# PlanNoa/video_super_resolution

Hardware: AMD Instinct MI355X
Metric: HR frames/sec, 1080p->4K x4 VSR (LR 540x960 -> 2160x3840), VSR.forward end-to-end (higher is better)
Workload: dtype f16

## Files before the change

### __graft_entry__.py

```python
import os

os.environ.setdefault("MIOPEN_FIND_MODE", "2")
os.environ.setdefault("MIOPEN_DEBUG_ENABLE_AI_IMMED_MODE_FALLBACK", "0")
os.environ.setdefault("MIOPEN_LOG_LEVEL", "2")
import subprocess
import sys

ROOT = os.path.dirname(os.path.abspath(__file__))
if ROOT not in sys.path:
    sys.path.insert(0, ROOT)


def build() -> None:
    from video_super_resolution_amd import _lib
    _lib.build(verbose=True)
    subprocess.check_call(["make", "-s", "-C", os.path.join(ROOT, "oracle"), "_build/liboracle_native.so"])
    import video_super_resolution_amd
    missing = [s for s in _lib.declared_symbols() if not hasattr(_lib.load(), s)]
    if missing:
        raise RuntimeError(f"libvsr_hip.so lacks {missing}")
    xmissing = [s for s in _lib.declared_symbols() + _lib.declared_symbols(xcheck=True) if not hasattr(_lib.load_xcheck(), s)]
    if xmissing:
        raise RuntimeError(f"libvsr_hip_xcheck.so lacks {xmissing}")
    s3missing = [s for s in _lib.declared_symbols(s3=True) if not hasattr(_lib.load_s3(), s)]
    if s3missing:
        raise RuntimeError(f"libvsr_hip_s3.so lacks {s3missing}")
    s3tmissing = [s for s in _lib.declared_symbols(s3t=True) if not hasattr(_lib.load_s3t(), s)]
    if s3tmissing:
        raise RuntimeError(f"libvsr_hip_s3t.so lacks {s3tmissing}")
    s3pmissing = [s for s in _lib.declared_symbols(s3p=True) if not hasattr(_lib.load_s3p(), s)]
    if s3pmissing:
        raise RuntimeError(f"libvsr_hip_s3p.so lacks {s3pmissing}")
    s3fmissing = [s for s in _lib.declared_symbols(s3f=True) if not hasattr(_lib.load_s3f(), s)]
    if s3fmissing:
        raise RuntimeError(f"libvsr_hip_s3f.so lacks {s3fmissing}")
    yuvmissing = [s for s in _lib.declared_symbols(yuv=True) if not hasattr(_lib.load_yuv(), s)]
    if yuvmissing:
        raise RuntimeError(f"libvsr_hip_yuv.so lacks {yuvmissing}")
    metricmissing = [s for s in _lib.declared_symbols(metric=True) if not hasattr(_lib.load_metric(), s)]
    if metricmissing:
        raise RuntimeError(f"libvsr_hip_metric.so lacks {metricmissing}")
    optmissing = [s for s in _lib.declared_symbols(opt=True) if not hasattr(_lib.load_opt(), s)]
    if optmissing:
        raise RuntimeError(f"libvsr_hip_opt.so lacks {optmissing}")
    lossmissing = [s for s in _lib.declared_symbols(loss=True) if not hasattr(_lib.load_loss(), s)]
    if lossmissing:
        raise RuntimeError(f"libvsr_hip_loss.so lacks {lossmissing}")
    resizemissing = [s for s in _lib.declared_symbols(resize=True) if not hasattr(_lib.load_resize(), s)]
    if resizemissing:
        raise RuntimeError(f"libvsr_hip_resize.so lacks {resizemissing}")
    warpmissing = [s for s in _lib.declared_symbols(warp=True) if not hasattr(_lib.load_warp(), s)]
    if warpmissing:
        raise RuntimeError(f"libvsr_hip_warp.so lacks {warpmissing}")
    scenemissing = [s for s in _lib.declared_symbols(scene=True) if not hasattr(_lib.load_scene(), s)]
    if scenemissing:
        raise RuntimeError(f"libvsr_hip_scene.so lacks {scenemissing}")
    hgimissing = [s for s in _lib.declared_symbols(hgi=True) if not hasattr(_lib.load_hgi(), s)]
    if hgimissing:
        raise RuntimeError(f"libvsr_hip_hgi.so lacks {hgimissing}")
    msssimmissing = [s for s in _lib.declared_symbols(msssim=True) if not hasattr(_lib.load_msssim(), s)]
    if msssimmissing:
        raise RuntimeError(f"libvsr_hip_msssim.so lacks {msssimmissing}")
    pixmissing = [s for s in _lib.declared_symbols(pix=True) if not hasattr(_lib.load_pix(), s)]
    if pixmissing:
        raise RuntimeError(f"libvsr_hip_pix.so lacks {pixmissing}")
    patchmissing = [s for s in _lib.declared_symbols(patch=True) if not hasattr(_lib.load_patch(), s)]
    if patchmissing:
        raise RuntimeError(f"libvsr_hip_patch.so lacks {patchmissing}")
    deintmissing = [s for s in _lib.declared_symbols(deint=True) if not hasattr(_lib.load_deint(), s)]
    if deintmissing:
        raise RuntimeError(f"libvsr_hip_deint.so lacks {deintmissing}")
    cellmissing = [s for s in _lib.declared_symbols(cell=True) if not hasattr(_lib.load_cell(), s)]
    if cellmissing:
        raise RuntimeError(f"libvsr_hip_cell.so lacks {cellmissing}")


def smoke() -> None:
    import numpy as np
    import torch
    from oracle import native, vsr_oracle
    from video_super_resolution_amd import SRProjectionModule, ops
    from video_super_resolution_amd.weights import fill_module_

    assert torch.cuda.is_available(), "smoke() needs cuda:0"
    torch.cuda.set_device(0)
    rs = np.random.RandomState(0)
    img = rs.randn(1, 3, 32, 48).astype(np.float32)
    flow = (rs.randn(1, 2, 32, 48) * 4).astype(np.float32)
    got = ops.resample2d(torch.from_numpy(img).cuda(), torch.from_numpy(flow).cuda()).cpu().numpy()
    assert np.array_equal(got, native.resample2d(img, flow)), "flow warp differs from the oracle"

    from video_super_resolution_amd import frames as F
    red = rs.randint(0, 256, (2, 20, 24)).astype(np.int64)
    rgb = np.zeros((2, 20, 24, 3), dtype=np.float32)
    rgb[..., 0] = red
    cells = F.cell_stats(torch.from_numpy(rgb).cuda(), luma4=(1.0, 0.0, 0.0, 0.0)).cpu().numpy()
    act = np.zeros_like(red)
    act[:, :, :-1] += np.abs(red[:, :, :-1] - red[:, :, 1:])
    act[:, :-1] += np.abs(red[:, :-1] - red[:, 1:])
    assert cells.shape == (2, 2, 2, 2) and cells[0, 0, 0, 0] == act[0, :16, :16].sum() and cells[1, 1, 1, 0] == act[1, 16:, 16:].sum(), \
        "cell activity differs from the sum it restates"
    assert not cells[0, :, :, 1].any() and cells[1, :, :, 1].sum() == np.abs(red[1] - red[0]).sum(), "cell temporal sums differ"

    sr = fill_module_(SRProjectionModule().eval(), seed=0, prefix="model.")
    x = torch.from_numpy(rs.randint(0, 256, (8, 3, 10, 12)).astype(np.float32))
    with torch.no_grad():
        ref = vsr_oracle.sr_forward({k: v for k, v in sr.state_dict().items()}, x).numpy()
    sr = sr.cuda()
    errs = {}
    for precision, bar in (("fp32", 1e-3), ("fp16", 5e-3)):
        sr.precision = precision
        out = sr(x.cuda()).cpu().numpy()
        errs[precision] = np.abs(out - ref).max() / np.abs(ref).max()
        assert errs[precision] < bar, f"SR forward ({precision}) differs from the oracle: {errs[precision]}"
    print(f"smoke ok: warp bit-exact, SR forward rel err fp32 {errs['fp32']:.2e}, fp16/MFMA {errs['fp16']:.2e}")


if __name__ == "__main__":
    build()
    if len(sys.argv) > 1 and sys.argv[1] == "smoke":
        smoke()
```

### video_super_resolution_amd/_lib.py

```python
from __future__ import annotations

import ctypes
import os
import re
import subprocess

import torch

_PKG = os.path.dirname(os.path.abspath(__file__))
_ROOT = os.path.dirname(_PKG)
LIB_PATH = os.path.join(_PKG, "libvsr_hip.so")
XLIB_PATH = os.path.join(_PKG, "libvsr_hip_xcheck.so")
HEADER_PATH = os.path.join(_ROOT, "include", "vsr_hip.h")
XHEADER_PATH = os.path.join(_ROOT, "include", "vsr_hip_xcheck.h")
_lib = None
_xlib = None


def _side(name: str, prefix: str, abi: int, has_query: bool) -> tuple:
    return (os.path.join(_PKG, f"libvsr_hip_{name}.so"), os.path.join(_ROOT, "include", f"vsr_hip_{name}.h"), prefix, abi, has_query)


_SIDE = {"grad": _side("grad", "vsr_grad", 1, False), "s3": _side("s3", "vsr_s3", 1, True), "s3t": _side("s3t", "vsr_s3t", 1, True),
         "s3p": _side("s3p", "vsr_s3p", 1, True), "s3f": _side("s3f", "vsr_s3f", 1, True), "yuv": _side("yuv", "vsr_yuv", 1, False),
         "metric": _side("metric", "vsr_metric", 1, False), "opt": _side("opt", "vsr_opt", 1, False), "loss": _side("loss", "vsr_loss", 1, False),
         "resize": _side("resize", "vsr_resize", 1, False), "warp": _side("warp", "vsr_warp", 1, False),
         "scene": _side("scene", "vsr_scene", 1, False), "hgi": _side("hgi", "vsr_hgi", 1, False),
         "msssim": _side("msssim", "vsr_msssim", 1, False), "pix": _side("pix", "vsr_pix", 1, False),
         "patch": _side("patch", "vsr_patch", 1, False), "deint": _side("deint", "vsr_deint", 1, False),
         "cell": _side("cell", "vsr_cell", 1, False)}
(GLIB_PATH, GHEADER_PATH), (S3LIB_PATH, S3HEADER_PATH), (S3TLIB_PATH, S3THEADER_PATH), (S3PLIB_PATH, S3PHEADER_PATH), \
    (S3FLIB_PATH, S3FHEADER_PATH), (YUVLIB_PATH, YUVHEADER_PATH), (METRICLIB_PATH, METRICHEADER_PATH), (OPTLIB_PATH, OPTHEADER_PATH), \
    (LOSSLIB_PATH, LOSSHEADER_PATH), (RESIZELIB_PATH, RESIZEHEADER_PATH), (WARPLIB_PATH, WARPHEADER_PATH), (SCENELIB_PATH, SCENEHEADER_PATH), \
    (HGILIB_PATH, HGIHEADER_PATH), (MSSSIMLIB_PATH, MSSSIMHEADER_PATH), (PIXLIB_PATH, PIXHEADER_PATH), (PATCHLIB_PATH, PATCHHEADER_PATH), \
    (DEINTLIB_PATH, DEINTHEADER_PATH), (CELLLIB_PATH, CELLHEADER_PATH) = (row[:2] for row in _SIDE.values())
_gradlib = _s3lib = _s3tlib = _s3plib = _s3flib = _yuvlib = _metriclib = _optlib = _losslib = _resizelib = _warplib = _scenelib = _hgilib = _msssimlib = _pixlib = _patchlib = _deintlib = _celllib = None
_use_x = os.environ.get("VSR_USE_XCHECK", "0") == "1" or bool(os.environ.get("VSR_TUNING", "").strip())


class VsrHipError(RuntimeError):
    pass


def build(verbose: bool = False) -> str:
    cmd = ["make", "-j4", "-C", os.path.join(_PKG, "csrc")]
    if not verbose:
        cmd.insert(1, "-s")
    subprocess.check_call(cmd)
    return LIB_PATH


def declared_symbols(xcheck: bool = False, grad: bool = False, s3: bool = False, s3t: bool = False, s3p: bool = False, s3f: bool = False,
                     yuv: bool = False, metric: bool = False, opt: bool = False, loss: bool = False, resize: bool = False,
                     warp: bool = False, scene: bool = False, hgi: bool = False, msssim: bool = False, pix: bool = False,
                     patch: bool = False, deint: bool = False, cell: bool = False) -> list:
    side = [name for name, on in (("grad", grad), ("s3", s3), ("s3t", s3t), ("s3p", s3p), ("s3f", s3f), ("yuv", yuv), ("metric", metric),
                                  ("opt", opt), ("loss", loss), ("resize", resize), ("warp", warp), ("scene", scene), ("hgi", hgi),
                                  ("msssim", msssim), ("pix", pix), ("patch", patch), ("deint", deint), ("cell", cell)) if on]
    with open(_SIDE[side[-1]][1] if side else XHEADER_PATH if xcheck else HEADER_PATH) as f:
        text = re.sub(r"/\*.*?\*/", "", f.read(), flags=re.S)
    return sorted(set(re.findall(r"\b(vsr_[a-z0-9_]+)\s*\(", text)))


def _dlopen(path: str) -> ctypes.CDLL:
    if not os.path.exists(path):
        raise VsrHipError(
            f"{path} is missing: build it with `python -c 'import __graft_entry__ as g; g.build()'` "
            "(there is no CPU fallback for the device path)")
    return ctypes.CDLL(path)


def _open(path: str) -> ctypes.CDLL:
    lib = _dlopen(path)
    lib.vsr_last_error.restype = ctypes.c_char_p
    lib.vsr_last_route.restype = ctypes.c_char_p
    for fn in ("vsr_sr_query", "vsr_train_corr_dw_ws_floats", "vsr_train_prelu_bwd_ws_floats"):
        getattr(lib, fn).restype = ctypes.c_size_t
    if lib.vsr_abi_version() != 3:
        raise VsrHipError(f"{os.path.basename(path)}: ABI version mismatch")
    return lib


def load_xcheck() -> ctypes.CDLL:
    global _xlib
    if _xlib is None:
        lib = _open(XLIB_PATH)
        for t in os.environ.get("VSR_TUNING", "").split(","):
            if t.strip():
                lib.vsr_conv2d_tuning(int(t))
        _xlib = lib
    return _xlib


def _load_side(name: str) -> ctypes.CDLL:
    cache = f"_{name}lib"
    if globals()[cache] is None:
        path, _, prefix, abi, has_query = _SIDE[name]
        lib = _dlopen(path)
        getattr(lib, prefix + "_last_error").restype = ctypes.c_char_p
        lib.vsr_last_error = getattr(lib, prefix + "_last_error")
        if has_query:
            getattr(lib, prefix + "_query").restype = ctypes.c_size_t
        if getattr(lib, prefix + "_abi_version")() != abi:
            raise VsrHipError(f"{os.path.basename(path)}: ABI version mismatch")
        globals()[cache] = lib
    return globals()[cache]


def load_grad() -> ctypes.CDLL:
    return _load_side("grad")


def load_s3() -> ctypes.CDLL:
    return _load_side("s3")


def load_s3t() -> ctypes.CDLL:
    return _load_side("s3t")


def load_s3p() -> ctypes.CDLL:
    return _load_side("s3p")


def load_s3f() -> ctypes.CDLL:
    return _load_side("s3f")


def load_yuv() -> ctypes.CDLL:
    return _load_side("yuv")


def load_metric() -> ctypes.CDLL:
    lib = _load_side("metric")
    lib.vsr_metric_ws_bytes.restype = ctypes.c_size_t
    return lib


class OptTensor(ctypes.Structure):
    _fields_ = [("p", ctypes.c_void_p), ("g", ctypes.c_void_p), ("m", ctypes.c_void_p), ("v", ctypes.c_void_p), ("n", ctypes.c_ulonglong)]


def load_opt() -> ctypes.CDLL:
    lib = _load_side("opt")
    lib.vsr_opt_plan_bytes.restype = lib.vsr_opt_norm_ws_bytes.restype = ctypes.c_size_t
    lib.vsr_opt_plan_bytes.argtypes = [ctypes.c_int, ctypes.POINTER(ctypes.c_ulonglong)]
    lib.vsr_opt_plan_fill.argtypes = [ctypes.c_void_p, ctypes.c_size_t, ctypes.c_int, ctypes.POINTER(OptTensor)]
    lib.vsr_opt_norm_ws_bytes.argtypes = [ctypes.c_void_p]
    lib.vsr_opt_adam_f32.argtypes = [ctypes.c_void_p] * 3 + [ctypes.c_float] * 7 + [ctypes.c_void_p]
    lib.vsr_opt_grad_norm.argtypes = [ctypes.c_void_p, ctypes.c_void_p, ctypes.c_double, ctypes.c_void_p, ctypes.c_void_p, ctypes.c_void_p]
    return lib


def load_loss() -> ctypes.CDLL:
    lib = _load_side("loss")
    lib.vsr_loss_ws_bytes.restype = ctypes.c_size_t
    lib.vsr_loss_ws_bytes.argtypes = [ctypes.c_int, ctypes.c_int]
    lib.vsr_loss_pixel_terms.argtypes = [ctypes.c_void_p] * 3 + [ctypes.c_int] * 2 + [ctypes.c_void_p] * 6
    return lib


def load_resize() -> ctypes.CDLL:
    lib = _load_side("resize")
    lib.vsr_resize_frames.argtypes = [ctypes.c_void_p] * 2 + [ctypes.c_int] * 5 + [ctypes.c_void_p, ctypes.c_void_p, ctypes.c_int] * 2 + \
        [ctypes.c_int, ctypes.c_void_p]
    return lib


def load_warp() -> ctypes.CDLL:
    lib = _load_side("warp")
    lib.vsr_warp_ws_bytes.restype = ctypes.c_size_t
    lib.vsr_warp_ws_bytes.argtypes = [ctypes.c_int] * 4
    lib.vsr_warp_error.argtypes = [ctypes.c_void_p] * 2 + [ctypes.c_int] * 7 + [ctypes.c_void_p] * 2 + [ctypes.c_int] + [ctypes.c_longlong] * 3 + \
        [ctypes.c_int] * 3 + [ctypes.c_void_p] * 5
    return lib


def load_scene() -> ctypes.CDLL:
    lib = _load_side("scene")
    lib.vsr_scene_ws_bytes.restype = ctypes.c_size_t
    lib.vsr_scene_ws_bytes.argtypes = [ctypes.c_int] * 3
    lib.vsr_scene_pair_sums.argtypes = [ctypes.c_void_p] * 2 + [ctypes.c_int] * 3 + [ctypes.c_void_p] * 4
    lib.vsr_scene_decide.argtypes = [ctypes.c_void_p, ctypes.c_int, ctypes.c_void_p, ctypes.c_double, ctypes.c_double, ctypes.c_void_p, ctypes.c_void_p]
    lib.vsr_scene_window.argtypes = [ctypes.c_void_p] * 4 + [ctypes.c_int] * 2 + [ctypes.c_void_p] * 4 + [ctypes.c_int] * 2 + [ctypes.c_void_p]
    return lib


def load_hgi() -> ctypes.CDLL:
    lib = _load_side("hgi")
    lib.vsr_hgi_workgroups.restype = ctypes.c_longlong
    lib.vsr_hgi_inception_f16.argtypes = [ctypes.c_void_p] + [ctypes.c_int] * 3 + [ctypes.c_void_p] * 2 + [ctypes.c_int] * 3 + \
        [ctypes.c_void_p, ctypes.c_void_p, ctypes.c_int] * 3 + [ctypes.c_int, ctypes.c_void_p] + [ctypes.c_int] * 4 + [ctypes.c_void_p]
    return lib


def load_msssim() -> ctypes.CDLL:
    lib = _load_side("msssim")
    lib.vsr_msssim_ws_bytes.restype = ctypes.c_size_t
    lib.vsr_msssim_ws_bytes.argtypes = [ctypes.c_int] * 5
    lib.vsr_msssim_frames.argtypes = [ctypes.c_void_p] * 2 + [ctypes.c_int] * 6 + [ctypes.c_void_p] * 5
    return lib


def load_pix() -> ctypes.CDLL:
    return _load_side("pix")


def load_patch() -> ctypes.CDLL:
    lib = _load_side("patch")
    lib.vsr_patch_gather.argtypes = [ctypes.c_void_p] + [ctypes.c_int] * 3 + [ctypes.c_void_p, ctypes.c_int, ctypes.c_void_p] + \
        [ctypes.c_int] * 4 + [ctypes.c_void_p] * 3
    return lib


class DeintPlane(ctypes.Structure):
    _fields_ = [("offset", ctypes.c_size_t), ("rows", ctypes.c_int), ("cols", ctypes.c_int), ("comps", ctypes.c_int)]


def load_deint() -> ctypes.CDLL:
    lib = _load_side("deint")
    lib.vsr_deint_frame.argtypes = [ctypes.c_void_p] * 4 + [ctypes.POINTER(DeintPlane)] + [ctypes.c_int] * 5 + [ctypes.c_void_p]
    return lib


def load_cell() -> ctypes.CDLL:
    lib = _load_side("cell")
    lib.vsr_cell_stats.argtypes = [ctypes.c_void_p] + [ctypes.c_int] * 3 + [ctypes.c_void_p] * 3
    return lib


def load() -> ctypes.CDLL:
    global _lib
    if _use_x:
        return load_xcheck()
    if _lib is None:
        _lib = _open(LIB_PATH)
    return _lib


class xcheck:

    def __enter__(self):
        global _use_x
        self._old, _use_x = _use_x, True
        return load_xcheck()

    def __exit__(self, *exc):
        global _use_x
        _use_x = self._old
        return False


Q_UTD_BLOB_BYTES, Q_UTD_STRIP_WIDTH, Q_UTD_S2_BLOB_BYTES, Q_UTD_S2_STRIP_WIDTH, Q_TAIL_S2_BLOB_BYTES = range(5)
Q_S3_BLOB_BYTES, Q_S3_STRIP_WIDTH = range(2)
Q_S3T_BLOB_BYTES, Q_S3T_BLOB_FOLD_BYTES, Q_S3T_STRIP_WIDTH = range(3)
Q_S3P_BLOB_BYTES, Q_S3P_STRIP_WIDTH = range(2)
Q_S3F_BLOB_BYTES, Q_S3F_STRIP_WIDTH = range(2)


def check(rc: int, what: str = "", lib=None) -> None:
    if rc != 0:
        libs = [lib] if lib is not None else [l for l in (load(), _lib, _xlib) if l is not None]
        msgs = []
        for l in libs:
            m = l.vsr_last_error().decode("utf-8", "replace")
            if m and m not in msgs:
                msgs.append(m)
        raise VsrHipError(f"{what or 'vsr'} failed ({rc}): {' | '.join(msgs)}")


def dptr(t: torch.Tensor, dtype=torch.float32) -> ctypes.c_void_p:
    if not t.is_cuda:
        raise VsrHipError("device path called with a CPU tensor (no CPU fallback exists)")
    if t.dtype != dtype:
        raise VsrHipError(f"expected {dtype}, got {t.dtype}")
    if not t.is_contiguous():
        raise VsrHipError("tensor must be contiguous")
    return ctypes.c_void_p(t.data_ptr())


def optr(t, dtype=torch.float32):
    return ctypes.c_void_p(0) if t is None else dptr(t, dtype)


_raw_stream = getattr(torch._C, "_cuda_getCurrentRawStream", None)


def raw_stream(index=None) -> int:
    if _raw_stream is not None:
        return _raw_stream(torch._C._cuda_getDevice() if index is None else index)
    return torch.cuda.current_stream(index).cuda_stream


def stream() -> ctypes.c_void_p:
    return ctypes.c_void_p(raw_stream())


def _first_cuda_tensor(objs):
    for o in objs:
        if isinstance(o, torch.Tensor):
            if o.is_cuda:
                return o
        elif isinstance(o, (list, tuple)):
            t = _first_cuda_tensor(o)
            if t is not None:
                return t
    return None


def on_device(fn):
    import functools

    @functools.wraps(fn)
    def wrapped(*args, **kwargs):
        t = _first_cuda_tensor(args)
        if t is None:
            t = _first_cuda_tensor(tuple(kwargs.values()))
        if t is None or t.device.index == torch.cuda.current_device():
            return fn(*args, **kwargs)
        with torch.cuda.device(t.device):
            return fn(*args, **kwargs)
    return wrapped


def cf(v: float) -> ctypes.c_float:
    return ctypes.c_float(float(v))


class _ChainStage(ctypes.Structure):
    _fields_ = [("inp", ctypes.c_void_p * 2), ("w", ctypes.c_void_p * 2), ("ldw", ctypes.c_int * 2), ("w_prev", ctypes.c_void_p),
                ("ldw_prev", ctypes.c_int), ("bias", ctypes.c_void_p), ("cmap", ctypes.c_void_p), ("slope", ctypes.c_float),
                ("out", ctypes.c_void_p)]


class Chain1x1(ctypes.Structure):
    _fields_ = [("nstages", ctypes.c_int), ("stage", _ChainStage * 3)]


_ROUTE_BATCH = os.environ.get("VSR_ROUTE_BATCH", "1") != "0"


class route_batch:

    def __init__(self, num: int, den: int):
        self.num, self.den = int(num), int(den)
        self.on = self.den > 0 and self.num > 0 and self.num != self.den and _ROUTE_BATCH

    def __enter__(self):
        if self.on:
            check(load().vsr_conv2d_route_batch(self.num, self.den), "conv2d_route_batch")
        return self

    def __exit__(self, *exc):
        if self.on:
            load().vsr_conv2d_route_batch(0, 0)
        return False


class serial_streams:
    on = False

    def __init__(self, enable: bool = True):
        self.enable = bool(enable)

    def __enter__(self):
        self._old, serial_streams.on = serial_streams.on, serial_streams.on or self.enable
        return self

    def __exit__(self, *exc):
        serial_streams.on = self._old
        return False


class EventTimer:

    def __init__(self):
        self.enabled = False
        self.only = None
        self._pairs = {}

    def reset(self):
        self._pairs = {}

# ... 47 lines not shown
```

### video_super_resolution_amd/csrc/conv_igemm.hip

```cpp
#include "conv_common.h"
#include "conv_kwalk.h"
#include "conv_patch.h"

namespace {

using vsrc::h8;
using vsrc::h4;
using vsrc::f4;
using vsrc::BM;
using vsrc::ConvP;
using vsrc::sw_off;
using vsrc::u4;
using vsrc::u2;
using vsrc::dma16;
using vsrc::patch_epilogue;
using vsrc::patch_epilogue_act;
using vsrc::patch_pixoff;
using vsrc::stage_patch;
using vsrc::patch_pieces;
using vsrc::stage_patch_cached;
using vsrc::PT_H;
using vsrc::PT_W;

struct C0 { static constexpr int value = 0; };
struct C1 { static constexpr int value = 1; };
struct C2 { static constexpr int value = 2; };
struct C3 { [[maybe_unused]] static constexpr int value = 3; };
struct C4 { [[maybe_unused]] static constexpr int value = 4; };


template <int BN, int ACT>
__device__ __forceinline__ void gather_store(const ConvP& p, const f4 (&acc)[BN / 16][2], long long M, long long m0, int co0, int tid, int zsplit,
                                             int ph, int oy_off, int ox_off) {
    constexpr int MT = BN / 16;
    const int lane = tid & 63, wv = tid >> 6, l15 = lane & 15, g = lane >> 4;
    if (p.splits > 1) {
#pragma unroll
        for (int nt = 0; nt < 2; ++nt) {
            const long long m = m0 + 32 * wv + 16 * nt + l15;
            if (m >= M) continue;
            float* wsp = p.ws + (((size_t)zsplit * (p.nphase > 1 ? 4 : 1) + ph) * M + m) * p.cout_pad + co0;
#pragma unroll
            for (int mt = 0; mt < MT; ++mt) *reinterpret_cast<f4*>(wsp + 16 * mt + 4 * g) = acc[mt][nt];
        }
        return;
    }
    f4 bz[MT];
#pragma unroll
    for (int mt = 0; mt < MT; ++mt)
        bz[mt] = p.bias ? *reinterpret_cast<const f4*>(p.bias + co0 + 16 * mt + 4 * g) : f4{0.0f, 0.0f, 0.0f, 0.0f};
    const bool vec_ok = (p.out_coff & 3) == 0 && (p.out_ld & 3) == 0;
    const unsigned HoWo = (unsigned)(p.Ho * p.Wo);
#pragma unroll
    for (int nt = 0; nt < 2; ++nt) {
        const long long m = m0 + 32 * wv + 16 * nt + l15;
        if (m >= M) continue;
        const int n = (int)((unsigned)m / HoWo);
        const int rem = (int)((unsigned)m - (unsigned)n * HoWo);
        const int oy = rem / p.Wo, ox = rem - oy * p.Wo;
        _Float16* dst = p.out + (((size_t)n * p.outH + oy * p.oy_mul + oy_off) * p.outW + ox * p.ox_mul + ox_off) * p.out_ld +
                        p.out_coff;
#pragma unroll
        for (int mt = 0; mt < MT; ++mt) {
            const int c = co0 + 16 * mt + 4 * g;
            if (c >= p.cout) continue;
            float v[4];
#pragma unroll
            for (int r = 0; r < 4; ++r) {
                float t = acc[mt][nt][r] + bz[mt][r];
                if (ACT == 1) t = fmaxf(t, 0.0f);
                else if (ACT == 2) t = t >= 0.0f ? t : t * p.slope;
                v[r] = t;
            }
            if (vec_ok && c + 4 <= p.cout) {
                *reinterpret_cast<h4*>(dst + c) = h4{(_Float16)v[0], (_Float16)v[1], (_Float16)v[2], (_Float16)v[3]};
            } else {
#pragma unroll
                for (int r = 0; r < 4; ++r)
                    if (c + r < p.cout) dst[c + r] = (_Float16)v[r];
            }
        }
    }
}

#if VSR_X
template <int BN, bool STEM = false>
__global__ void __launch_bounds__(256) k_conv_igemm(const ConvP p) {
    constexpr int MT = BN / 16;
    constexpr int A_HALF = BN * 64;
    constexpr int B_HALF = BM * 64;
    constexpr int STAGE = 2 * (A_HALF + B_HALF);
    constexpr int A_PIECES = A_HALF / 16;
    constexpr int AP = (A_PIECES + 255) / 256;
    extern __shared__ __attribute__((aligned(16))) unsigned char smem[];
    auto As = [&](int b, int hf) __attribute__((always_inline)) { return smem + b * STAGE + hf * (A_HALF + B_HALF); };
    auto Bs = [&](int b, int hf) __attribute__((always_inline)) { return smem + b * STAGE + hf * (A_HALF + B_HALF) + A_HALF; };
    u4* const tab = reinterpret_cast<u4*>(smem + 2 * STAGE);

    const int tid = threadIdx.x, lane = tid & 63, wv = tid >> 6;
    const int l15 = lane & 15, g = lane >> 4;
    const long long M = (long long)p.N * p.Ho * p.Wo;
    const long long m0 = (long long)blockIdx.x * BM;
    const int co0 = blockIdx.y * BN;
    const int nchunk = STEM ? 1 : p.cin >> 5;
    const int npair = STEM ? p.kh : p.kh * p.kw * nchunk;
    const int nk_all = (npair + 1) >> 1;
    const vsrc::KRange kr = vsrc::k_range(p, blockIdx.z, nk_all);
    const int ph = kr.ph, zsplit = kr.zsplit, pad_y = kr.pad_y, pad_x = kr.pad_x, oy_off = kr.oy_off, ox_off = kr.ox_off;
    const int ks_per = kr.ks_per, ks0 = kr.ks0, nk = kr.nk;
    const _Float16* const wpk = kr.wpk;

    const __amdgpu_buffer_rsrc_t w_rsrc = vsrc::kwalk_w_rsrc(p, wpk, npair), in_rsrc = vsrc::kwalk_in_rsrc(p);

    vsrc::build_kwalk<STEM>(p, tab, tid, ks0, nk, npair, nchunk, vsrc::kwalk_entries(ks_per, vsrc::KWALK_FIRST_LOOKAHEAD));

    const int bchunk = tid & 3;
    const int brow[2] = {tid >> 2, (tid + 256) >> 2};
    int piy0[2], pix0[2];
    unsigned pbase[2];
    bool xok0[2], xok1[2];
#pragma unroll
    for (int r = 0; r < 2; ++r) {
        const vsrc::PixOrigin o = vsrc::pixel_origin<STEM>(p, m0 + brow[r], M, pad_y, pad_x, bchunk);
        piy0[r] = o.piy0; pix0[r] = o.pix0; pbase[r] = o.pbase;
        xok0[r] = (unsigned)pix0[r] < (unsigned)p.W;
        xok1[r] = (unsigned)(pix0[r] + 1) < (unsigned)p.W;
    }
    unsigned wlane[AP];
#pragma unroll
    for (int ap = 0; ap < AP; ++ap) wlane[ap] = tid + 256 * ap < A_PIECES ? (unsigned)(co0 * 64 + (tid + 256 * ap) * 16) : 0x40000000u;

    u4 ra[2][2][AP], rb[2][2][2];
    __syncthreads();
    int q = 0;
    u4 en[2] = {tab[0], tab[1]};
    auto gload = [&](auto setc) __attribute__((always_inline)) {
        constexpr int S = decltype(setc)::value;
#pragma unroll
        for (int hf = 0; hf < 2; ++hf) {
            const u4 e = en[hf];
#pragma unroll
            for (int ap = 0; ap < AP; ++ap) ra[S][hf][ap] = __builtin_amdgcn_raw_buffer_load_b128(w_rsrc, wlane[ap] + e[3], 0, 0);
#pragma unroll
            for (int r = 0; r < 2; ++r) {
                const bool rowok = (unsigned)(piy0[r] + (int)e[1]) < (unsigned)p.H;
                if (STEM) {
                    const u2 t0 = __builtin_amdgcn_raw_buffer_load_b64(in_rsrc, rowok && xok0[r] ? pbase[r] + e[0] : 0xFFFFFFFFu, 0, 0);
                    const u2 t1 = __builtin_amdgcn_raw_buffer_load_b64(in_rsrc, rowok && xok1[r] ? pbase[r] + e[0] + 8u : 0xFFFFFFFFu, 0, 0);
                    rb[S][hf][r] = u4{t0[0], t0[1], t1[0], t1[1]};
                } else {
                    const bool ok = rowok && (unsigned)(pix0[r] + (int)e[2]) < (unsigned)p.W;
                    rb[S][hf][r] = __builtin_amdgcn_raw_buffer_load_b128(in_rsrc, ok ? pbase[r] + e[0] : 0xFFFFFFFFu, 0, 0);
                }
            }
        }
// ... 61 lines not shown
    else if (p.act == 1) gather_store<BN, 1>(p, acc, M, m0, co0, tid, zsplit, ph, oy_off, ox_off);
    else gather_store<BN, 2>(p, acc, M, m0, co0, tid, zsplit, ph, oy_off, ox_off);
}
#endif


template <int BN, bool STEM = false, int D = 3>
__global__ void __launch_bounds__(256) k_conv_igemm_d(const ConvP p) {
    constexpr int MT = BN / 16;
    constexpr int A_HALF = BN * 64;
    constexpr int STAGE = 2 * A_HALF;
    constexpr int A_PIECES = A_HALF / 16;
    constexpr int AP = (A_PIECES + 255) / 256;
    extern __shared__ __attribute__((aligned(16))) unsigned char smem[];
    auto As = [&](int b, int hf) __attribute__((always_inline)) { return smem + b * STAGE + hf * A_HALF; };
    u4* const tab = reinterpret_cast<u4*>(smem + 2 * STAGE);

    const int tid = threadIdx.x, lane = tid & 63, wv = tid >> 6;
    const int l15 = lane & 15, g = lane >> 4;
    const long long M = (long long)p.N * p.Ho * p.Wo;
    const long long m0 = (long long)blockIdx.x * BM;
    const int co0 = blockIdx.y * BN;
    const int nchunk = STEM ? 1 : p.cin >> 5;
    const int npair = STEM ? p.kh : p.kh * p.kw * nchunk;
    const int nk_all = (npair + 1) >> 1;
    const vsrc::KRange kr = vsrc::k_range(p, blockIdx.z, nk_all);
    const int ph = kr.ph, zsplit = kr.zsplit, pad_y = kr.pad_y, pad_x = kr.pad_x, oy_off = kr.oy_off, ox_off = kr.ox_off;
    const int ks_per = kr.ks_per, ks0 = kr.ks0, nk = kr.nk;
    const _Float16* const wpk = kr.wpk;

    const __amdgpu_buffer_rsrc_t w_rsrc = vsrc::kwalk_w_rsrc(p, wpk, npair), in_rsrc = vsrc::kwalk_in_rsrc(p);

    vsrc::build_kwalk<STEM>(p, tab, tid, ks0, nk, npair, nchunk, vsrc::kwalk_entries(ks_per, vsrc::kwalk_gather_lookahead(D)));

    int piy0[2], pix0[2];
    unsigned pbase[2];
    bool xok0[2], xok1[2];
#pragma unroll
    for (int r = 0; r < 2; ++r) {
        const int row = 32 * wv + 16 * r + l15;
        const vsrc::PixOrigin o = vsrc::pixel_origin<STEM>(p, m0 + row, M, pad_y, pad_x, g);
        piy0[r] = o.piy0; pix0[r] = o.pix0; pbase[r] = o.pbase;
        xok0[r] = (unsigned)pix0[r] < (unsigned)p.W;
        xok1[r] = (unsigned)(pix0[r] + 1) < (unsigned)p.W;
    }

    u4 ra[D][2][AP], rb[D][2][2];
    unsigned wlane[AP];
#pragma unroll
    for (int ap = 0; ap < AP; ++ap) wlane[ap] = tid + 256 * ap < A_PIECES ? (unsigned)(co0 * 64 + (tid + 256 * ap) * 16) : 0x40000000u;
    __syncthreads();
    int q = 0;
    u4 en[2] = {tab[0], tab[1]};
    auto gload = [&](auto setc, auto setb) __attribute__((always_inline)) {
        constexpr int S = decltype(setc)::value, SB = decltype(setb)::value;
#pragma unroll
        for (int hf = 0; hf < 2; ++hf) {
            const u4 e = en[hf];
#pragma unroll
            for (int ap = 0; ap < AP; ++ap) ra[S][hf][ap] = __builtin_amdgcn_raw_buffer_load_b128(w_rsrc, wlane[ap] + e[3], 0, 0);
#pragma unroll
            for (int r = 0; r < 2; ++r) {
                const bool rowok = (unsigned)(piy0[r] + (int)e[1]) < (unsigned)p.H;
                if (STEM) {
                    const u2 t0 = __builtin_amdgcn_raw_buffer_load_b64(in_rsrc, rowok && xok0[r] ? pbase[r] + e[0] : 0xFFFFFFFFu, 0, 0);
                    const u2 t1 = __builtin_amdgcn_raw_buffer_load_b64(in_rsrc, rowok && xok1[r] ? pbase[r] + e[0] + 8u : 0xFFFFFFFFu, 0, 0);
                    rb[SB][hf][r] = u4{t0[0], t0[1], t1[0], t1[1]};
                } else {
                    const bool ok = rowok && (unsigned)(pix0[r] + (int)e[2]) < (unsigned)p.W;
                    rb[SB][hf][r] = __builtin_amdgcn_raw_buffer_load_b128(in_rsrc, ok ? pbase[r] + e[0] : 0xFFFFFFFFu, 0, 0);
                }
            }
        }
        q += 2;
        en[0] = tab[q];
        en[1] = tab[q + 1];
    };
    auto lstore = [&](int buf, auto setc) __attribute__((always_inline)) {
        constexpr int S = decltype(setc)::value;
#pragma unroll
        for (int hf = 0; hf < 2; ++hf) {
#pragma unroll
            for (int ap = 0; ap < AP; ++ap) {
                const int piece = tid + 256 * ap;
                if (piece < A_PIECES) *reinterpret_cast<u4*>(As(buf, hf) + sw_off(piece >> 2, piece & 3)) = ra[S][hf][ap];
            }
        }
    };

    f4 acc[MT][2];
#pragma unroll
    for (int mt = 0; mt < MT; ++mt)
#pragma unroll
        for (int nt = 0; nt < 2; ++nt) acc[mt][nt] = f4{0.0f, 0.0f, 0.0f, 0.0f};

    gload(C0{}, C0{});
    lstore(ks0 & 1, C0{});
    gload(C1{}, C1{});
    if constexpr (D == 5) {
        gload(C2{}, C2{});
        gload(C3{}, C3{});
    }
    __syncthreads();
    auto body = [&](int ks, auto cur, auto nxt, auto nw) __attribute__((always_inline)) {
        constexpr int BC = decltype(cur)::value;
        const int buf = ks & 1;
        h8 af[2][MT];
#pragma unroll
        for (int mt = 0; mt < MT; ++mt) af[0][mt] = *reinterpret_cast<const h8*>(As(buf, 0) + sw_off(16 * mt + l15, g));
        __builtin_amdgcn_sched_barrier(0);
        gload(nw, nw);
        __builtin_amdgcn_sched_barrier(0);
#pragma unroll
        for (int mt = 0; mt < MT; ++mt) af[1][mt] = *reinterpret_cast<const h8*>(As(buf, 1) + sw_off(16 * mt + l15, g));
        __builtin_amdgcn_sched_barrier(0);
        if (ks < nk) {
#pragma unroll
            for (int hf = 0; hf < 2; ++hf) {
                h8 bf[2];
#pragma unroll
                for (int nt = 0; nt < 2; ++nt) bf[nt] = __builtin_bit_cast(h8, rb[BC][hf][nt]);
#pragma unroll
                for (int mt = 0; mt < MT; ++mt)
#pragma unroll
                    for (int nt = 0; nt < 2; ++nt)
                        acc[mt][nt] = __builtin_amdgcn_mfma_f32_16x16x32_f16(af[hf][mt], bf[nt], acc[mt][nt], 0, 0, 0);
            }
        }
        lstore(buf ^ 1, nxt);
        __syncthreads();
    };
    if constexpr (D == 5) {
        for (int ks = ks0; ks < nk; ks += 5) {
            body(ks, C0{}, C1{}, C4{});
            body(ks + 1, C1{}, C2{}, C0{});
            body(ks + 2, C2{}, C3{}, C1{});
            body(ks + 3, C3{}, C4{}, C2{});
            body(ks + 4, C4{}, C0{}, C3{});
        }
    } else {
        for (int ks = ks0; ks < nk; ks += 3) {
            body(ks, C0{}, C1{}, C2{});
            body(ks + 1, C1{}, C2{}, C0{});
            body(ks + 2, C2{}, C0{}, C1{});
        }
    }

    if (p.splits > 1 || p.act == 0) gather_store<BN, 0>(p, acc, M, m0, co0, tid, zsplit, ph, oy_off, ox_off);
    else if (p.act == 1) gather_store<BN, 1>(p, acc, M, m0, co0, tid, zsplit, ph, oy_off, ox_off);
    else gather_store<BN, 2>(p, acc, M, m0, co0, tid, zsplit, ph, oy_off, ox_off);
}


constexpr int C1_MAX_CHUNKS = 8;
template <int NCH>
__global__ void __launch_bounds__(512) k_conv1x1_stream(const ConvP p) {
    extern __shared__ __attribute__((aligned(16))) unsigned char wsm[];
    const int tid = threadIdx.x, lane = tid & 63, wv = tid >> 6;
    const int l15 = lane & 15, g = lane >> 4;
    const long long M = (long long)p.N * p.Ho * p.Wo;
    const int rows = NCH * p.cout_pad;
    for (int q = tid; q < rows * 4; q += 512)
        *reinterpret_cast<uint4*>(wsm + sw_off(q >> 2, q & 3)) = *reinterpret_cast<const uint4*>(p.wpk + (size_t)q * 8);
    float* const bsm = reinterpret_cast<float*>(wsm + (size_t)rows * 64);
    for (int q = tid; q < p.cout_pad; q += 512) bsm[q] = (p.bias && q < p.cout) ? p.bias[q] : 0.0f;
    __syncthreads();
    const int ntile = min(p.cout_pad >> 4, 2 * ((p.cout + 31) >> 5));
    const long long nblk = (M + 255) / 256;
    h8 bf[NCH][2], nx[NCH][2];
    auto fetch = [&](long long blk, h8 (&dst)[NCH][2]) __attribute__((always_inline)) {
#pragma unroll
        for (int nt = 0; nt < 2; ++nt) {
            const long long m = blk * 256 + 32 * wv + 16 * nt + l15;
            const _Float16* src = p.in + (size_t)(m < M ? m : M - 1) * p.in_ld + p.in_coff + 8 * g;
#pragma unroll
            for (int c = 0; c < NCH; ++c) dst[c][nt] = *reinterpret_cast<const h8*>(src + 32 * c);
        }
    };
    if ((long long)blockIdx.x < nblk) fetch(blockIdx.x, nx);
    for (long long blk = blockIdx.x; blk < nblk; blk += gridDim.x) {
        const long long mbase = blk * 256 + 32 * wv;
#pragma unroll
        for (int c = 0; c < NCH; ++c)
#pragma unroll
            for (int nt = 0; nt < 2; ++nt) bf[c][nt] = nx[c][nt];
        if (blk + gridDim.x < nblk) fetch(blk + gridDim.x, nx);
        const float nslope = p.act == 1 ? 0.0f : (p.act == 2 ? p.slope : 1.0f);
        const bool vec_ok = (p.out_coff & 7) == 0 && (p.out_ld & 7) == 0;
        int t = 0;
        for (; t + 1 < ntile; t += 2) {
            const int rowA = 16 * t + 8 * (l15 >> 2) + (l15 & 3);
            h8 a0[NCH], a1[NCH];
#pragma unroll
            for (int c = 0; c < NCH; ++c) {
                a0[c] = *reinterpret_cast<const h8*>(wsm + sw_off(c * p.cout_pad + rowA, g));
                a1[c] = *reinterpret_cast<const h8*>(wsm + sw_off(c * p.cout_pad + rowA + 4, g));
            }
            const int c0 = 16 * t + 8 * g;
            const f4 b0 = *reinterpret_cast<const f4*>(bsm + c0), b1 = *reinterpret_cast<const f4*>(bsm + c0 + 4);
            f4 acc[2][2];
#pragma unroll
            for (int nt = 0; nt < 2; ++nt) { acc[0][nt] = b0; acc[1][nt] = b1; }
#pragma unroll
            for (int c = 0; c < NCH; ++c)
#pragma unroll
                for (int nt = 0; nt < 2; ++nt) {
                    acc[0][nt] = __builtin_amdgcn_mfma_f32_16x16x32_f16(a0[c], bf[c][nt], acc[0][nt], 0, 0, 0);
                    acc[1][nt] = __builtin_amdgcn_mfma_f32_16x16x32_f16(a1[c], bf[c][nt], acc[1][nt], 0, 0, 0);
                }
            const bool full = vec_ok && c0 + 8 <= p.cout;
#pragma unroll
            for (int nt = 0; nt < 2; ++nt) {
                const long long m = mbase + 16 * nt + l15;
                float v[8];
#pragma unroll
                for (int r = 0; r < 8; ++r) {
                    const float x = acc[r >> 2][nt][r & 3];
                    v[r] = fmaxf(x, 0.0f) + nslope * fminf(x, 0.0f);
                }
                _Float16* dst = p.out + (size_t)(m < M ? m : 0) * p.out_ld + p.out_coff + c0;
                if (m < M && full) {
                    *reinterpret_cast<h8*>(dst) = h8{(_Float16)v[0], (_Float16)v[1], (_Float16)v[2], (_Float16)v[3],
                                                     (_Float16)v[4], (_Float16)v[5], (_Float16)v[6], (_Float16)v[7]};
                } else if (m < M) {
#pragma unroll
                    for (int r = 0; r < 8; ++r)
                        if (c0 + r < p.cout) dst[r] = (_Float16)v[r];
                }
            }
        }
        if (t < ntile) {
            h8 a0[NCH];
#pragma unroll
            for (int c = 0; c < NCH; ++c) a0[c] = *reinterpret_cast<const h8*>(wsm + sw_off(c * p.cout_pad + 16 * t + l15, g));
            const int c0 = 16 * t + 4 * g;
            const f4 b0 = *reinterpret_cast<const f4*>(bsm + c0);
            f4 acc[2] = {b0, b0};
#pragma unroll
            for (int c = 0; c < NCH; ++c)
#pragma unroll
                for (int nt = 0; nt < 2; ++nt) acc[nt] = __builtin_amdgcn_mfma_f32_16x16x32_f16(a0[c], bf[c][nt], acc[nt], 0, 0, 0);
            const bool full = (p.out_coff & 3) == 0 && (p.out_ld & 3) == 0 && c0 + 4 <= p.cout;
#pragma unroll
            for (int nt = 0; nt < 2; ++nt) {
                const long long m = mbase + 16 * nt + l15;
                float v[4];
#pragma unroll
                for (int r = 0; r < 4; ++r) v[r] = fmaxf(acc[nt][r], 0.0f) + nslope * fminf(acc[nt][r], 0.0f);
                _Float16* dst = p.out + (size_t)(m < M ? m : 0) * p.out_ld + p.out_coff + c0;
                if (m < M && full) {
                    *reinterpret_cast<h4*>(dst) = h4{(_Float16)v[0], (_Float16)v[1], (_Float16)v[2], (_Float16)v[3]};
                } else if (m < M) {
#pragma unroll
                    for (int r = 0; r < 4; ++r)
                        if (c0 + r < p.cout) dst[r] = (_Float16)v[r];
                }
            }
        }
    }
}

#if VSR_X
constexpr int C1T_SLOT = 32 * 256;
__global__ void __launch_bounds__(256) k_conv1x1_t(const ConvP p) {
    constexpr int NCH = 4;
    extern __shared__ __attribute__((aligned(16))) unsigned char wsm[];
    const int tid = threadIdx.x, lane = tid & 63, wv = __builtin_amdgcn_readfirstlane(tid >> 6);
    const int l15 = lane & 15, g = lane >> 4;
    const long long M = (long long)p.N * p.Ho * p.Wo;
    const int rows = NCH * p.cout_pad;
    for (int q = tid; q < rows * 4; q += 256)
        *reinterpret_cast<uint4*>(wsm + sw_off(q >> 2, q & 3)) = *reinterpret_cast<const uint4*>(p.wpk + (size_t)q * 8);
    float* const bsm = reinterpret_cast<float*>(wsm + (size_t)rows * 64);
    for (int q = tid; q < p.cout_pad; q += 256) bsm[q] = (p.bias && q < p.cout) ? p.bias[q] : 0.0f;
    unsigned char* const slots = wsm + (size_t)rows * 64 + (size_t)p.cout_pad * 4 + (size_t)wv * 2 * C1T_SLOT;
    __syncthreads();
    const long long nblk = (M + 127) / 128;
    const __amdgpu_buffer_rsrc_t in_rsrc = __builtin_amdgcn_make_buffer_rsrc(
        const_cast<_Float16*>(p.in), 0, (int)((size_t)M * p.in_ld * 2), 0x00020000);
    const __amdgpu_buffer_rsrc_t out_rsrc = __builtin_amdgcn_make_buffer_rsrc(p.out, 0, (int)((size_t)M * p.out_ld * 2), 0x00020000);
    const int dq = lane >> 4, ds = lane & 15;
    auto fetch = [&](long long blk, int slot) __attribute__((always_inline)) {
        const long long m0 = blk * 128 + 32 * wv;
#pragma unroll
        for (int k = 0; k < 8; ++k) {
            const int pl = 4 * k + dq;
            const long long m = m0 + pl;
            const unsigned off = m < M ? (unsigned)(((size_t)m * p.in_ld + p.in_coff) * 2 + ((ds ^ (pl & 15)) << 4)) : 0xFFFFFFFFu;
            dma16(in_rsrc, slots + slot * C1T_SLOT + 1024 * k, off);
        }
    };
    const float nslope = p.act == 1 ? 0.0f : (p.act == 2 ? p.slope : 1.0f);
    const int ngroup = (p.cout + 127) >> 7;
    auto store_group = [&](const unsigned char* tile, long long mbase, int grp) __attribute__((always_inline)) {
        const int npair = min(4, (p.cout_pad - 128 * grp) >> 5);
        const int ch = 128 * grp + 8 * ds;
        const bool ch_ok = ch + 8 <= p.cout && ds < 4 * npair;
#pragma unroll
        for (int k = 0; k < 8; ++k) {
            const int pl = 4 * k + dq;
            const long long m = mbase + pl;
            const u4 v = *reinterpret_cast<const u4*>(tile + pl * 256 + ((ds ^ (pl & 15)) << 4));
            const unsigned off = (ch_ok && m < M) ? (unsigned)(((size_t)m * p.out_ld + p.out_coff + ch) * 2) : 0xFFFFFFFFu;
            __builtin_amdgcn_raw_buffer_store_b128(v, out_rsrc, off, 0, 0);
        }
        asm volatile("s_waitcnt lgkmcnt(0)" ::: "memory");
    };
    int cur = 0;
    bool have_prev = false;
    long long prev_mbase = 0;
    if ((long long)blockIdx.x >= nblk) return;
    fetch(blockIdx.x, 0);
    for (long long blk = blockIdx.x; blk < nblk; blk += gridDim.x, cur ^= 1) {
        unsigned char* const img = slots + cur * C1T_SLOT;
        unsigned char* const oth = slots + (cur ^ 1) * C1T_SLOT;
        asm volatile("s_waitcnt vmcnt(0)" ::: "memory");
        h8 bf[NCH][2];
#pragma unroll
        for (int nt = 0; nt < 2; ++nt)
#pragma unroll
            for (int c = 0; c < NCH; ++c) {
                const int pl = 16 * nt + l15;
                bf[c][nt] = *reinterpret_cast<const h8*>(img + pl * 256 + (((4 * c + g) ^ (pl & 15)) << 4));
            }
        asm volatile("s_waitcnt lgkmcnt(0)" ::: "memory");
        if (have_prev) store_group(oth, prev_mbase, ngroup - 1);
        fetch(blk + gridDim.x, cur ^ 1);
        const long long mbase = blk * 128 + 32 * wv;
        for (int grp = 0; grp < ngroup; ++grp) {
            const int npair = min(4, (p.cout_pad - 128 * grp) >> 5);
            for (int tp = 0; tp < npair; ++tp) {
                const int t = 8 * grp + 2 * tp;
                const int rowA = 16 * t + 8 * (l15 >> 2) + (l15 & 3);
                h8 a0[NCH], a1[NCH];
#pragma unroll
                for (int c = 0; c < NCH; ++c) {
                    a0[c] = *reinterpret_cast<const h8*>(wsm + sw_off(c * p.cout_pad + rowA, g));
                    a1[c] = *reinterpret_cast<const h8*>(wsm + sw_off(c * p.cout_pad + rowA + 4, g));
                }
                const int c0 = 16 * t + 8 * g;
                const f4 b0 = *reinterpret_cast<const f4*>(bsm + c0), b1 = *reinterpret_cast<const f4*>(bsm + c0 + 4);
                f4 acc[2][2];
#pragma unroll
                for (int nt = 0; nt < 2; ++nt) { acc[0][nt] = b0; acc[1][nt] = b1; }
#pragma unroll
                for (int c = 0; c < NCH; ++c)
#pragma unroll
                    for (int nt = 0; nt < 2; ++nt) {
                        acc[0][nt] = __builtin_amdgcn_mfma_f32_16x16x32_f16(a0[c], bf[c][nt], acc[0][nt], 0, 0, 0);
                        acc[1][nt] = __builtin_amdgcn_mfma_f32_16x16x32_f16(a1[c], bf[c][nt], acc[1][nt], 0, 0, 0);
                    }
#pragma unroll
                for (int nt = 0; nt < 2; ++nt) {
                    float v[8];
#pragma unroll
                    for (int r = 0; r < 8; ++r) {
                        const float x = acc[r >> 2][nt][r & 3];
                        v[r] = fmaxf(x, 0.0f) + nslope * fminf(x, 0.0f);
                    }
                    const int pl = 16 * nt + l15;
                    *reinterpret_cast<h8*>(img + pl * 256 + (((4 * tp + g) ^ (pl & 15)) << 4)) =
                        h8{(_Float16)v[0], (_Float16)v[1], (_Float16)v[2], (_Float16)v[3], (_Float16)v[4], (_Float16)v[5], (_Float16)v[6], (_Float16)v[7]};
                }
            }
            asm volatile("" ::: "memory");
            if (grp + 1 < ngroup) store_group(img, mbase, grp);
        }
        have_prev = true;
        prev_mbase = mbase;
    }
    store_group(slots + (cur ^ 1) * C1T_SLOT, prev_mbase, ngroup - 1);
    asm volatile("s_waitcnt vmcnt(0)" ::: "memory");
}
#endif




template <int MT>
__global__ void __launch_bounds__(256) k_conv_patch(const ConvP p) {
    extern __shared__ __attribute__((aligned(16))) unsigned char psm[];
    const int PH = PT_H + p.kh - 1, PW = PT_W + p.kw - 1;
    const int ntap = p.kh * p.kw;
    unsigned char* const patch = psm;
    const int tid = threadIdx.x, lane = tid & 63, wv = tid >> 6;
    const int l15 = lane & 15, g = lane >> 4;
    const vsrc::PatchTile t0 = vsrc::patch_tile<PT_H, PT_W>(p, p.Wo);
    const int n = t0.n, oy0 = t0.oy0, ox0 = t0.ox0, iy0 = t0.iy0, ix0 = t0.ix0;
    const int co0 = blockIdx.z * 16 * MT;
    const int nchunk = p.cin >> 5;

    f4 acc[MT][4];
#pragma unroll
    for (int mt = 0; mt < MT; ++mt)
#pragma unroll
        for (int t = 0; t < 4; ++t) acc[mt][t] = f4{0.0f, 0.0f, 0.0f, 0.0f};
    int poff[4];
#pragma unroll
    for (int t = 0; t < 4; ++t) poff[t] = (2 * wv + (t >> 1)) * PW + 16 * (t & 1) + l15;
    auto wfrag = [&](int tap, int ch, int mt) __attribute__((always_inline)) {
        return *reinterpret_cast<const h8*>(p.wpk + ((size_t)(tap * nchunk + ch) * p.cout_pad + co0 + 16 * mt + l15) * 32 + 8 * g);
    };
    for (int ch = 0; ch < nchunk; ++ch) {
        __syncthreads();
        stage_patch(p, patch, n, ch, iy0, ix0, PH, PW, tid);
        h8 af[MT], afn[MT];
#pragma unroll
        for (int mt = 0; mt < MT; ++mt) af[mt] = wfrag(0, ch, mt);
        __syncthreads();
        int tap = 0;
        for (int ky = 0; ky < p.kh; ++ky)
            for (int kx = 0; kx < p.kw; ++kx, ++tap) {
                const int tn = tap + 1 < ntap ? tap + 1 : tap;
// ... 547 lines not shown
        p.outH == Ho && p.outW == Wo && (cin >> 5) <= C1_MAX_CHUNKS && (size_t)(cin >> 5) * cout_pad * 64 <= 128 * 1024 && cout_pad > 64 && Mr >= 65536 &&
        !g_sw.no_patch) {
#if VSR_X
        if (g_c1t_mode >= 1 && cin == 128 && (p.cout & 7) == 0 && (p.out_ld & 7) == 0 && (p.out_coff & 7) == 0 && c1t_lds(p) <= 160 * 1024 &&
            (unsigned long long)M * p.in_ld * 2 < kGatherLimit && (unsigned long long)M * p.out_ld * 2 < kGatherLimit && p.cout <= 256)
            return ConvRoute{Kind::conv1x1_t, 0, 0, 1, false};
#endif
        return ConvRoute{Kind::conv1x1_stream, 0, 0, 1, false};
    }
    if (tile_ok) return plan_tile(p, M, Mr, nk_all, 1, tile_bn, tile_splits, has_ws, ws_bytes);
    const unsigned gxr = vsr::cdiv(Mr, BM);
    const bool wide = (cout_pad & 127) == 0 && !g_sw.first_gather && !g_sw.wide_never && (g_sw.wide_always || (long long)gxr * (cout_pad / 128) >= 128);
    const int bn = wide ? 128 : (cout_pad & 63) == 0 ? 64 : ((cout_pad & 31) == 0 ? 32 : 16);
    const long long wgs = (long long)gxr * (cout_pad / bn);
    int splits = 1;
    if (has_ws && wgs < g_splitk_fill && nk_all >= 8) splits = clamp_splits((int)((g_splitk_fill * 2 + wgs - 1) / wgs), nk_all, 1, M, Mr, cout_pad, has_ws, ws_bytes);
    return ConvRoute{Kind::gather, bn, 0, splits, g_sw.first_gather};
}

static ConvRoute plan_stem(const ConvP& p, int Nr, bool, size_t) {
    const long long Mr = (long long)Nr * p.Ho * p.Wo;
    if (!g_sw.no_patch && p.kh == 7 && p.kw == 7 && p.stride == 1 && p.pad_y == 3 && p.pad_x == 3 && p.cout == 128 && p.cout_pad == 128 && p.Ho == p.H &&
        p.Wo == p.W && (p.out_ld & 7) == 0 && (p.out_coff & 7) == 0 && (unsigned long long)p.N * p.H * p.W * 8 < (1ull << 31) && Mr >= 65536 &&
        (long long)p.N * vsr::cdiv(p.Wo, ST_C) * vsr::cdiv(p.Ho, ST_R) < (1ll << 30))
        return ConvRoute{Kind::stem7_rows, 0, 0, 1, false};
    return ConvRoute{Kind::gather_stem, (p.cout_pad & 63) == 0 ? 64 : ((p.cout_pad & 31) == 0 ? 32 : 16), 0, 1, g_sw.first_gather};
}

static ConvRoute plan_deconv(const ConvP& p, int Nr, bool has_ws, size_t ws_bytes) {
    const int cout_pad = p.cout_pad, H = p.H, W = p.W;
    const long long M = (long long)p.N * H * W, Mr = (long long)Nr * H * W;
    const int nk_all = (4 * (p.cin >> 5) + 1) >> 1;
    const bool patch_on = !g_sw.no_patch && !g_sw.first_gather;
    if (patch_on && cout_pad <= 32 && (long long)H * W >= 8192 && H >= 4 && W >= 16 && p.N <= 65535 &&
        (unsigned long long)(PT_H + 18) * W * p.in_ld * 2 < (1ull << 31))
        return ConvRoute{Kind::deconv4s2_patch, 0, 0, 1, false};
    int tile_splits = 1;
    const int tile_bn = tile_choice(p, Mr, nk_all, 4, &tile_splits);
    if (g_tile_mode >= 1 && patch_on && (cout_pad & 63) == 0 && (g_tile_mode >= 3 || tile_bn != 0))
        return plan_tile(p, M, Mr, nk_all, 4, tile_bn, tile_splits, has_ws, ws_bytes);
    const int bn = (cout_pad & 63) == 0 ? 64 : ((cout_pad & 31) == 0 ? 32 : 16);
    const long long wgs = (long long)vsr::cdiv(Mr, BM) * (cout_pad / bn) * 4;
    int splits = 1;
    if (has_ws && wgs < 128 && nk_all >= 8) splits = clamp_splits((int)(256 / wgs), nk_all, 4, M, Mr, cout_pad, has_ws, ws_bytes);
    return ConvRoute{Kind::gather, bn, 0, splits, g_sw.first_gather};
}

static void route_name(const ConvRoute& r, const ConvP& p) {
    const char* dc = p.nphase > 1 ? "deconv4s2 " : "";
    switch (r.kind) {
    case Kind::gather: vsr::route(r.splits > 1 ? "%sgather<%d>+splitk%d" : "%sgather<%d>", dc, r.bn, r.splits); break;
    case Kind::gather_stem: vsr::route("gather<%d,stem>", r.bn); break;
    case Kind::tile: vsr::route(r.splits > 1 ? "%stile<%d>+splitk%d" : "%stile<%d>", dc, r.bn, r.splits); break;
    case Kind::deconv4s2_patch: vsr::route("deconv4s2_patch"); break;
    case Kind::stem7_rows: vsr::route("stem7_rows"); break;
    case Kind::patch_pf: vsr::route("patch_pf<%d,%d>", p.kh, r.mt); break;
    case Kind::patch_lw: vsr::route("patch_lw<%d,%d>", p.kh, r.mt); break;
    case Kind::patch_r8: vsr::route("patch_r8<%d,%d>", p.kh, r.mt); break;
    case Kind::patch: vsr::route("patch<%d>", r.mt); break;
    case Kind::patch_rows: vsr::route("patch_rows<%d>", p.kh); break;
    case Kind::conv1x1_stream: vsr::route("conv1x1_stream<%d>", p.cin >> 5); break;
    case Kind::conv1x1_t: vsr::route("conv1x1_t"); break;
    }
}

static const char* launch_name(const ConvRoute& r, const ConvP& p) {
    const bool dc = p.nphase > 1;
    switch (r.kind) {
    case Kind::gather: return dc ? "deconv4s2_nhwc_f16" : "conv2d_nhwc_f16";
    case Kind::gather_stem: return "conv2d_stem_f16";
    case Kind::tile: return dc ? "deconv4s2_nhwc_f16/tile" : "conv2d_nhwc_f16/tile";
    case Kind::deconv4s2_patch: return "deconv4s2_nhwc_f16/patch";
    case Kind::stem7_rows: return "conv2d_stem_f16/rows";
    case Kind::patch_pf: return "conv2d_nhwc_f16/patch_pf";
    case Kind::patch_lw: return "conv2d_nhwc_f16/patch_lw";
    case Kind::patch_r8: return "conv2d_nhwc_f16/patch_r8";
    case Kind::patch:
    case Kind::patch_rows: return "conv2d_nhwc_f16/patch";
    case Kind::conv1x1_stream: return "conv2d_nhwc_f16/1x1";
    case Kind::conv1x1_t: return "conv2d_nhwc_f16/1x1t";
    }
    return "conv2d";
}

static int launch_gather_wide(const ConvP& p, dim3 grid, hipStream_t st);
template <bool STEM>
static int launch_gather_bn(const ConvP& p, const ConvRoute& r, dim3 grid, hipStream_t st) {
#if VSR_X
    if (r.first_build)
        return r.bn == 64 ? launch_gather_lds<64, STEM>(p, grid, st) : r.bn == 32 ? launch_gather_lds<32, STEM>(p, grid, st) : launch_gather_lds<16, STEM>(p, grid, st);
#endif
    if (!STEM && r.bn == 128) return launch_gather_wide(p, grid, st);
    return r.bn == 64 ? launch_gather<64, STEM>(p, grid, st) : r.bn == 32 ? launch_gather<32, STEM>(p, grid, st) : launch_gather<16, STEM>(p, grid, st);
}

typedef void (*conv_kernel_t)(const ConvP);
struct BigLds {
    conv_kernel_t k;
    unsigned long long raised;
};
static void raise_lds(BigLds& e) { vsr::raise_lds_limit_once(e.raised, e.k, 160 * 1024); }

static int launch_route(const ConvP& p, const ConvRoute& r, hipStream_t st) {
    const long long M = (long long)p.N * p.Ho * p.Wo;
    const int kh = p.kh, nph = p.nphase > 1 ? p.nphase : 1;
    int rc = VSR_OK;
    switch (r.kind) {
    case Kind::gather:
    case Kind::gather_stem: {
        const dim3 grid(vsr::cdiv(M, BM), p.cout_pad / r.bn, nph * r.splits);
        rc = r.kind == Kind::gather ? launch_gather_bn<false>(p, r, grid, st) : launch_gather_bn<true>(p, r, grid, st);
        break;
    }
    case Kind::tile:
        rc = vsrc::launch_conv_tile(p, r.bn, st);
        break;
    case Kind::deconv4s2_patch:
        hipLaunchKernelGGL(k_deconv4s2_patch, dim3(vsr::cdiv(p.H, PT_H) * vsr::cdiv(p.W, PT_W), p.N, p.cout_pad / 16), dim3(256), (PT_H + 2) * (PT_W + 2) * 64, st, p);
        break;
    case Kind::stem7_rows: {
        const int tiles_x = (int)vsr::cdiv(p.Wo, ST_C), tiles_y = (int)vsr::cdiv(p.Ho, ST_R);
        const long long ntiles = (long long)p.N * tiles_x * tiles_y;
        const unsigned grid1 = (unsigned)(ntiles < 256 * 2 ? ntiles : 256 * 2);
        hipLaunchKernelGGL(k_stem7_rows, dim3(grid1), dim3(256), 0, st, p, tiles_x, tiles_y, (int)ntiles);
        break;
    }
    case Kind::patch_pf:
        rc = vsrc::launch_conv_patch_pf(p, r.mt, st);
        break;
    case Kind::patch_lw:
    case Kind::patch_r8: {
        static BigLds lw[4] = {{k_conv_patch_lw<3, 4>, 0}, {k_conv_patch_lw<3, 2>, 0}, {k_conv_patch_lw<5, 2>, 0}, {k_conv_patch_lw<7, 2>, 0}};
        static BigLds r8[4][2] = {{{k_conv_patch_r8<3, 2>, 0}, {k_conv_patch_r8<3, 1>, 0}}, {{k_conv_patch_r8<5, 2>, 0}, {k_conv_patch_r8<5, 1>, 0}},
                                  {{k_conv_patch_r8<7, 2>, 0}, {k_conv_patch_r8<7, 1>, 0}}, {{k_conv_patch_r8<11, 2>, 0}, {k_conv_patch_r8<11, 1>, 0}}};
        const bool is_lw = r.kind == Kind::patch_lw;
        BigLds& e = is_lw ? lw[r.mt == 4 ? 0 : 1 + kh_slot(kh)] : r8[kh_slot(kh)][2 - r.mt];
        static const int lw_lds[4] = {vsrc::P8Geom<3, 4>::LW_LDS, vsrc::P8Geom<3, 2>::LW_LDS, vsrc::P8Geom<5, 2>::LW_LDS, vsrc::P8Geom<7, 2>::LW_LDS};
        const int r8_patch = (P8_H + kh - 1) * (P8_W + p.kw - 1) * 64, r8_out = 4 * P8_R * 16 * 32 * r.mt;
        const int lds = is_lw ? lw_lds[r.mt == 4 ? 0 : 1 + kh_slot(kh)] : r8_patch > r8_out ? r8_patch : r8_out;
        if (lds > 64 * 1024) raise_lds(e);
        hipLaunchKernelGGL(e.k, dim3(vsr::cdiv(p.Ho, P8_H) * vsr::cdiv(p.Wo, P8_W), p.N, p.cout_pad / (16 * r.mt)), dim3(256), lds, st, p);
        break;
    }
    case Kind::patch:
    case Kind::patch_rows: {
        const int lds_patch = (PT_H + kh - 1) * (PT_W + p.kw - 1) * 64, lds_out = 4 * 4 * 16 * 32 * r.mt;
        static const conv_kernel_t ks[7] = {k_conv_patch<4>, k_conv_patch<2>, k_conv_patch_rows<3>, k_conv_patch_rows<5>, k_conv_patch_rows<7>,
                                            k_conv_patch_rows<11>, k_conv_patch<1>};
        const conv_kernel_t k = ks[r.kind == Kind::patch_rows ? 2 + kh_slot(kh) : r.mt == 4 ? 0 : r.mt == 2 ? 1 : 6];
        hipLaunchKernelGGL(k, dim3(vsr::cdiv(p.Ho, PT_H) * vsr::cdiv(p.Wo, PT_W), p.N, p.cout_pad / (16 * r.mt)), dim3(256), lds_patch > lds_out ? lds_patch : lds_out, st, p);
        break;
    }
    case Kind::conv1x1_stream: {
        static const conv_kernel_t k1[C1_MAX_CHUNKS] = {k_conv1x1_stream<1>, k_conv1x1_stream<2>, k_conv1x1_stream<3>, k_conv1x1_stream<4>,
                                                        k_conv1x1_stream<5>, k_conv1x1_stream<6>, k_conv1x1_stream<7>, k_conv1x1_stream<8>};
        const conv_kernel_t k = k1[(p.cin >> 5) - 1];
        const size_t k_lds = (size_t)(p.cin >> 5) * p.cout_pad * 64 + (size_t)p.cout_pad * 4;
        if (k_lds > 48 * 1024 &&
            hipFuncSetAttribute(reinterpret_cast<const void*>(k), hipFuncAttributeMaxDynamicSharedMemorySize, (int)k_lds) != hipSuccess)
            return vsr::fail(VSR_E_LAUNCH, "conv2d/1x1: cannot reserve %zu bytes of LDS", k_lds);
        const int per_cu = (int)((160 * 1024) / k_lds) < 2 ? 1 : 2;
        const long long nblk = (M + 255) / 256;
        hipLaunchKernelGGL(k, dim3((unsigned)(nblk < 256LL * per_cu ? nblk : 256LL * per_cu)), dim3(512), k_lds, st, p);
        break;
    }
    case Kind::conv1x1_t: {
#if VSR_X
        static BigLds t = {k_conv1x1_t, 0};
        raise_lds(t);
        const size_t t_lds = c1t_lds(p);
        const int per_cu = (int)((160 * 1024) / t_lds) < 2 ? 1 : 2;
        const long long nblk = (M + 127) / 128;
        hipLaunchKernelGGL(k_conv1x1_t, dim3((unsigned)(nblk < 256LL * per_cu ? nblk : 256LL * per_cu)), dim3(256), t_lds, st, p);
#endif
        break;
    }
    }
    if (rc) return rc;
    if (r.splits > 1) {
        rc = vsr::launched(launch_name(r, p));
        if (rc) return rc;
        hipLaunchKernelGGL(k_splitk_finish, dim3(vsr::cdiv(M * (p.cout_pad >> 2), 256), nph), dim3(256), 0, st, p);
    }
    return vsr::launched(launch_name(r, p));
}
static int launch_gather_wide(const ConvP& p, dim3 grid, hipStream_t st) { return launch_gather<128, false>(p, grid, st); }

static ConvP make_convp(const void* in, int in_ld, int in_coff, const void* w_packed, const float* bias, void* out, int out_ld, int out_coff, int N, int H,
                        int W, int cin, int Ho, int Wo, int cout, int cout_pad, int kh, int kw, int stride, int stride_x, int pad_y, int pad_x, int outH,
                        int outW, int oy_mul, int oy_off, int ox_mul, int ox_off, int act, float slope) {
    ConvP p = {};
    p.in = (const _Float16*)in; p.wpk = (const _Float16*)w_packed; p.bias = bias; p.out = (_Float16*)out;
    p.in_ld = in_ld; p.in_coff = in_coff; p.out_ld = out_ld; p.out_coff = out_coff;
    p.N = N; p.H = H; p.W = W; p.cin = cin; p.Ho = Ho; p.Wo = Wo; p.cout = cout; p.cout_pad = cout_pad;
    p.kh = kh; p.kw = kw; p.stride = stride; p.stride_x = stride_x > 0 ? stride_x : stride; p.pad_y = pad_y; p.pad_x = pad_x;
    p.outH = outH; p.outW = outW; p.oy_mul = oy_mul; p.oy_off = oy_off; p.ox_mul = ox_mul; p.ox_off = ox_off;
    p.act = act; p.slope = slope; p.ws = nullptr; p.splits = 1; p.nphase = 0;
    return p;
}
static ConvP make_stem(const void* in4, const void* w_packed, const float* bias, void* out, int out_ld, int out_coff, int N, int H, int W, int Ho, int Wo,
                       int cout, int cout_pad, int kh, int kw, int stride, int pad_y, int pad_x, int act, float slope) {
    return make_convp(in4, 4, 0, w_packed, bias, out, out_ld, out_coff, N, H, W, 32, Ho, Wo, cout, cout_pad, kh, kw, stride, 0, pad_y, pad_x, Ho, Wo, 1, 0, 1, 0,
                      act, slope);
}
static ConvP make_deconv(const void* in, int in_ld, int in_coff, const void* const* w_packed4, const float* bias, void* out, int out_ld, int out_coff, int N,
                         int H, int W, int cin, int cout, int cout_pad, int act, float slope) {
    ConvP p = make_convp(in, in_ld, in_coff, nullptr, bias, out, out_ld, out_coff, N, H, W, cin, H, W, cout, cout_pad, 2, 2, 1, 1, 0, 0, 2 * H, 2 * W, 2, 0, 2, 0,
                         act, slope);
    p.nphase = 4;
    for (int ph = 0; ph < 4; ++ph) {
        const int py = ph >> 1, px = ph & 1;
        p.wpk_ph[ph] = w_packed4 ? (const _Float16*)w_packed4[ph] : nullptr;
        p.pad_y_ph[ph] = py == 0 ? 1 : 0; p.pad_x_ph[ph] = px == 0 ? 1 : 0;
        p.oy_off_ph[ph] = py; p.ox_off_ph[ph] = px;
    }
    return p;
}

static int check_conv(const ConvP& p) {
    VSR_REQUIRE(p.N > 0 && p.H > 0 && p.W > 0 && p.Ho > 0 && p.Wo > 0 && p.cout > 0 && p.kh > 0 && p.kw > 0 && p.stride > 0, "conv2d: bad shape");
    VSR_REQUIRE(p.cin > 0 && (p.cin & 31) == 0, "conv2d: input channels %d must be padded to a multiple of 32", p.cin);
    VSR_REQUIRE((p.in_ld & 7) == 0 && (p.in_coff & 7) == 0 && p.in_coff + p.cin <= p.in_ld, "conv2d: input slice [%d,+%d) of %d channels", p.in_coff, p.cin, p.in_ld);
    VSR_REQUIRE(p.out_coff >= 0 && p.out_coff + p.cout <= p.out_ld, "conv2d: output slice [%d,+%d) of %d channels", p.out_coff, p.cout, p.out_ld);
    VSR_REQUIRE(p.cout_pad >= p.cout && (p.cout_pad & 15) == 0, "conv2d: cout_pad %d", p.cout_pad);
    VSR_REQUIRE((p.Ho - 1) * p.oy_mul + p.oy_off < p.outH && (p.Wo - 1) * p.ox_mul + p.ox_off < p.outW && p.oy_off >= 0 && p.ox_off >= 0,
                "conv2d: output window exceeds the destination tensor");
    VSR_REQUIRE(p.act >= 0 && p.act <= 2, "conv2d: activation %d", p.act);
    VSR_REQUIRE((unsigned long long)p.H * p.W * p.in_ld * 2 < kGatherLimit, "conv2d: one %dx%dx%d fp16 image exceeds the 4 GiB the kernels address", p.H, p.W, p.in_ld);
    return VSR_OK;
}
static int check_stem(const ConvP& p) {
    VSR_REQUIRE(p.N > 0 && p.H > 0 && p.W > 0 && p.Ho > 0 && p.Wo > 0 && p.cout > 0 && p.kh > 0 && p.kw > 0 && p.kw <= 8 && p.stride > 0, "conv2d_stem: bad shape");
    VSR_REQUIRE(p.out_coff >= 0 && p.out_coff + p.cout <= p.out_ld && p.cout_pad >= p.cout && (p.cout_pad & 15) == 0, "conv2d_stem: output slice");
    VSR_REQUIRE(p.act >= 0 && p.act <= 2, "conv2d_stem: activation %d", p.act);
    VSR_REQUIRE((unsigned long long)p.N * p.H * p.W * 8 < kGatherLimit, "conv2d_stem: input batch beyond the 4 GiB the kernel addresses");
    return VSR_OK;
}
static int check_deconv(const ConvP& p) {
    VSR_REQUIRE(p.N > 0 && p.H > 0 && p.W > 0 && p.cout > 0 && p.cin > 0 && (p.cin & 31) == 0, "deconv4s2: bad shape");
    VSR_REQUIRE((p.in_ld & 7) == 0 && (p.in_coff & 7) == 0 && p.in_coff + p.cin <= p.in_ld, "deconv4s2: input slice");
    VSR_REQUIRE(p.out_coff >= 0 && p.out_coff + p.cout <= p.out_ld && p.cout_pad >= p.cout && (p.cout_pad & 15) == 0, "deconv4s2: output slice");
    VSR_REQUIRE(p.act >= 0 && p.act <= 2, "deconv4s2: activation %d", p.act);
    VSR_REQUIRE((unsigned long long)p.H * p.W * p.in_ld * 2 < kGatherLimit, "deconv4s2: one %dx%dx%d fp16 image exceeds the 4 GiB the kernel addresses", p.H, p.W, p.in_ld);
    return VSR_OK;
}

template <class F>
static int for_sub_batches(const ConvP& p, size_t img_out, F&& run) {
    const unsigned long long img_in = (unsigned long long)p.H * p.W * p.in_ld;
    const int per = img_in * 2 * p.N >= kGatherLimit ? (int)((kGatherLimit - 1) / (img_in * 2)) : p.N;
    for (int n0 = 0; n0 < p.N; n0 += per) {
        ConvP q = p;
        q.in = p.in + (size_t)n0 * img_in; q.out = p.out + (size_t)n0 * img_out; q.N = p.N - n0 < per ? p.N - n0 : per;
        const int rc = run(q);
        if (rc) return rc;
    }
    return VSR_OK;
}

enum Entry { kConv = 0, kStem = 1, kDeconv = 2 };
struct EntryDef {
    int (*check)(const ConvP&);
    ConvRoute (*plan)(const ConvP&, int Nr, bool has_ws, size_t ws_bytes);
    const char* too_many;
};
static const EntryDef kEntries[3] = {
    {check_conv, plan_conv, "conv2d: %lld output pixels exceed the kernels' 32-bit pixel index"},
    {check_stem, plan_stem, "conv2d_stem: %lld output pixels exceed the kernels' 32-bit pixel index"},
    {check_deconv, plan_deconv, "deconv4s2: %lld output pixels per phase exceed the kernel's 32-bit pixel index"}};

static int plan_named(Entry entry, const ConvP& p, bool has_ws, size_t ws_bytes, ConvRoute* r) {
    const long long M = (long long)p.N * p.Ho * p.Wo;
    if (M >= (1ll << 31)) return vsr::fail(VSR_E_ARG, kEntries[entry].too_many, M);
    *r = kEntries[entry].plan(p, vsr::route_batch(p.N), has_ws, ws_bytes);
    route_name(*r, p);
    return VSR_OK;
}

static int run_planned(Entry entry, ConvP& p, void* splitk_ws, size_t splitk_ws_bytes, vsr_stream_t stream) {
    ConvRoute r;
    const int rc = plan_named(entry, p, splitk_ws != nullptr, splitk_ws_bytes, &r);
    if (rc) return rc;
    p.splits = r.splits;
    p.ws = r.splits > 1 ? (float*)splitk_ws : nullptr;
    return launch_route(p, r, vsr::S(stream));
}

extern "C" {

#if VSR_X
int vsr_conv2d_tuning(int patch_mode) {
    const int old = g_patch_mode;
    if (patch_mode >= 9000) { g_pf_mode = patch_mode - 9000; return old; }
    if (patch_mode >= 8000) { g_gather_deep = patch_mode - 8000; return old; }
    if (patch_mode >= 7000) { g_c1t_mode = patch_mode - 7000; return old; }
    if (patch_mode >= 6000) { g_lw_mode = patch_mode - 6000; return old; }
    if (patch_mode >= 5000) { g_tile_splits = patch_mode - 5000; return old; }
    if (patch_mode >= 4000) { g_tile_bn = patch_mode - 4000; return old; }
    if (patch_mode >= 2000) { g_tile_mode = patch_mode - 2000; return old; }
    if (patch_mode >= 1000) {
        g_splitk_fill = patch_mode - 1000;
        return old;
    }
    g_patch_mode = patch_mode;
    g_sw = decode_patch_mode(patch_mode);
    return old;
}
#endif
// ... 61 lines not shown
```

### video_super_resolution_amd/csrc/conv_patch_pf.hip

```cpp
#include "conv_patch.h"

namespace {

using vsrc::ConvP;
using vsrc::f4;
using vsrc::h8;
using vsrc::P8_H;
using vsrc::P8_R;
using vsrc::P8_W;
using vsrc::sw_off;

typedef vsrc::u4 u4v;

template <int KH, int MT, int WPS>
__global__ void __launch_bounds__(256, WPS) k_conv_patch_pf(const ConvP p, int tiles_x, int tiles_y, int nwork) {
    typedef vsrc::P8Geom<KH, MT> G;
    constexpr int PH = G::PH, PW = G::PW, NPC = G::NPC, NWC = G::NWC, WTAP = G::WTAP;
    extern __shared__ __attribute__((aligned(16))) unsigned char psm[];
    unsigned char* const patch = psm;
    unsigned char* const wts = psm + G::WOFF;
    const int tid = threadIdx.x, lane = tid & 63, wv = __builtin_amdgcn_readfirstlane(tid >> 6);
    const int l15 = lane & 15, g = lane >> 4;
    const int nchunk = p.cin >> 5, nblk = p.cout_pad / (16 * MT);
    const int ry0 = P8_R * (wv >> 1), cx0 = 16 * (wv & 1);

    const __amdgpu_buffer_rsrc_t w_rsrc = __builtin_amdgcn_make_buffer_rsrc(
        const_cast<_Float16*>(p.wpk), 0, (int)((size_t)KH * KH * nchunk * p.cout_pad * 64), 0x00020000);
    int wdst[NWC];
    unsigned wsrc[NWC];
#pragma unroll
    for (int j = 0; j < NWC; ++j) {
        const int q = tid + 256 * j;
        const int row = q >> 2, slot = q & 3, tap = row / (16 * MT), r = row - tap * (16 * MT);
        const bool in = q * 16 < G::WBYTES;
        wdst[j] = in ? tap * WTAP + sw_off(r, slot) : -1;
        wsrc[j] = in ? (unsigned)(((size_t)tap * nchunk * p.cout_pad + r) * 64 + slot * 16) : 0xFFFFFFFFu;
    }

    f4 acc[P8_R][MT];
#pragma unroll
    for (int r = 0; r < P8_R; ++r)
#pragma unroll
        for (int mt = 0; mt < MT; ++mt) acc[r][mt] = f4{0.0f, 0.0f, 0.0f, 0.0f};

    u4v pf[NPC + NWC];
    unsigned poff[NPC];
    int pdst[NPC];
    struct Item { int n, oy0, ox0, co0, by; };
    auto decode = [&](int w) {
        Item it;
        const int blk = w % nblk, t = w / nblk;
        const int tx = t % tiles_x, t2 = t / tiles_x, ty = t2 % tiles_y;
        it.n = t2 / tiles_y;
        it.oy0 = ty * P8_H; it.ox0 = tx * P8_W; it.co0 = blk * 16 * MT;
        const int iy0 = it.oy0 - p.pad_y;
        it.by = iy0 > 0 ? iy0 : 0;
        return it;
    };
    auto issue = [&](const Item& it, int ch) __attribute__((always_inline)) {
        const __amdgpu_buffer_rsrc_t rs = vsrc::patch_rsrc_at(p, it.n, it.by);
#pragma unroll
        for (int k = 0; k < NPC; ++k) pf[k] = __builtin_amdgcn_raw_buffer_load_b128(rs, vsrc::cached_piece_off(poff[k], ch), 0, 0);
        const unsigned woff = (unsigned)(((size_t)ch * p.cout_pad + it.co0) * 64);
#pragma unroll
        for (int j = 0; j < NWC; ++j)
            pf[NPC + j] = __builtin_amdgcn_raw_buffer_load_b128(w_rsrc, wsrc[j] == 0xFFFFFFFFu ? 0xFFFFFFFFu : wsrc[j] + woff, 0, 0);
    };
    auto commit = [&]() __attribute__((always_inline)) {
#pragma unroll
        for (int k = 0; k < NPC; ++k)
            if (pdst[k] >= 0) *reinterpret_cast<u4v*>(patch + pdst[k]) = pf[k];
#pragma unroll
        for (int j = 0; j < NWC; ++j)
            if (wdst[j] >= 0) *reinterpret_cast<u4v*>(wts + wdst[j]) = pf[NPC + j];
    };

    int w = blockIdx.x;
    if (w >= nwork) return;
    Item cur = decode(w);
    vsrc::patch_pieces(p, cur.oy0 - p.pad_y, cur.ox0 - p.pad_x, PH, PW, tid, poff, pdst);
    issue(cur, 0);
    Item nxt = cur;
    int ch = 0;
    while (true) {
        __syncthreads();
        commit();
        __syncthreads();
        const bool last_chunk = ch + 1 == nchunk;
        const int w2 = last_chunk ? w + (int)gridDim.x : w;
        const bool have_next = !last_chunk || w2 < nwork;
        if (have_next) {
            if (last_chunk) {
                nxt = decode(w2);
                vsrc::patch_pieces(p, nxt.oy0 - p.pad_y, nxt.ox0 - p.pad_x, PH, PW, tid, poff, pdst);
            }
            issue(nxt, last_chunk ? 0 : ch + 1);
        }
#pragma unroll 1
        for (int kx = 0; kx < KH; ++kx) {
            h8 A[KH][MT];
#pragma unroll
            for (int ky = 0; ky < KH; ++ky)
#pragma unroll
                for (int mt = 0; mt < MT; ++mt)
                    A[ky][mt] = *reinterpret_cast<const h8*>(wts + (ky * KH + kx) * WTAP + sw_off(16 * mt + l15, g));
            const int px = cx0 + l15 + kx;
            const unsigned char* src = patch + (ry0 * PW + px) * 64 + ((g ^ ((px >> 1) & 3)) << 4);
#pragma unroll
            for (int pr = 0; pr < KH + P8_R - 1; ++pr) {
                const h8 bf = *reinterpret_cast<const h8*>(src + pr * PW * 64);
#pragma unroll
                for (int r = 0; r < P8_R; ++r) {
                    const int ky = pr - r;
                    if (ky < 0 || ky >= KH) continue;
#pragma unroll
                    for (int mt = 0; mt < MT; ++mt) acc[r][mt] = __builtin_amdgcn_mfma_f32_16x16x32_f16(A[ky][mt], bf, acc[r][mt], 0, 0, 0);
                }
            }
        }
        if (!last_chunk) { ++ch; continue; }
        __syncthreads();
        {
            const vsrc::WaveOut wo = vsrc::wave_out(p, cur.n, cur.oy0 + ry0, cur.ox0 + cx0);
            vsrc::patch_epilogue<MT, P8_R>(p, psm + wv * (P8_R * 16 * 32 * MT), cur.co0, lane, [&](int r, int mt) { return acc[r][mt]; },
                                           [&](int r, int li) { return r < wo.rows_ok && li < wo.cols_ok ? wo.wbase + r * wo.rstride + li * wo.cstride : -1ll; });
        }
        if (!have_next) break;
#pragma unroll
        for (int r = 0; r < P8_R; ++r)
#pragma unroll
            for (int mt = 0; mt < MT; ++mt) acc[r][mt] = f4{0.0f, 0.0f, 0.0f, 0.0f};
        cur = nxt; w = w2; ch = 0;
    }
}

template <int KH, int MT, int WPS>
int launch_pf(const ConvP& p, int N, hipStream_t stream) {
    typedef vsrc::P8Geom<KH, MT> G;
    static unsigned long long raised = 0;
    if (G::LDS > 64 * 1024) vsr::raise_lds_limit_once(raised, &k_conv_patch_pf<KH, MT, WPS>, 160 * 1024);
    const int tiles_x = (int)vsr::cdiv(p.Wo, P8_W), tiles_y = (int)vsr::cdiv(p.Ho, P8_H);
    const long long nwork = (long long)N * tiles_x * tiles_y * (p.cout_pad / (16 * MT));
    if (nwork >= (1ll << 30)) return vsr::fail(VSR_E_ARG, "conv2d/patch_pf: %lld work items", nwork);
    int per_cu = (160 * 1024) / G::LDS;
    if (per_cu > WPS) per_cu = WPS;
    if (per_cu < 1) per_cu = 1;
    const long long resident = 256LL * per_cu;
    const unsigned grid = (unsigned)(nwork < resident ? nwork : resident);
    hipLaunchKernelGGL((k_conv_patch_pf<KH, MT, WPS>), dim3(grid), dim3(256), G::LDS, stream, p, tiles_x, tiles_y, (int)nwork);
    return VSR_OK;
}

}

namespace vsrc {

bool patch_pf_has(int kh, int mt) { return (kh == 3 && (mt == 1 || mt == 2)) || (kh == 5 && mt == 1); }

int launch_conv_patch_pf(const ConvP& p, int mt, hipStream_t stream) {
    const int N = p.N;
    if (p.kh == 3 && mt == 1) return launch_pf<3, 1, 3>(p, N, stream);
    if (p.kh == 3 && mt == 2) return launch_pf<3, 2, 2>(p, N, stream);
    if (p.kh == 5 && mt == 1) return launch_pf<5, 1, 2>(p, N, stream);
    return vsr::fail(VSR_E_ARG, "conv2d/patch_pf: no build for %dx%d with %d out-channels per workgroup", p.kh, p.kw, 16 * mt);
}

}
```

### video_super_resolution_amd/igemm.py

```python
from __future__ import annotations

import torch
import torch.nn as nn

from . import _lib as L

import ctypes

ACT_NONE, ACT_RELU, ACT_LEAKY = 0, 1, 2
_WS_BYTES = 64 << 20
_MAX_SHAPES = 4
_ws = {}


def _splitk_ws(device) -> torch.Tensor:
    key = (device.type, device.index, L.raw_stream(device.index))
    if key not in _ws:
        _ws[key] = torch.empty(_WS_BYTES // 4, dtype=torch.float32, device=device)
    return _ws[key]


def pad32(c: int) -> int:
    return (c + 31) // 32 * 32

# ... 133 lines not shown
        Ho = (H + 2 * self.pad - self.kh) // self.stride + 1
        Wo = (W + 2 * self.pad - self.kw) // self.stride + 1
        if out is None:
            cp = pad32(out_coff + self.cout)
            out = cached_zeros(self, "out", (N, Ho, Wo, cp), x4.device) if cp != out_coff + self.cout else \
                torch.empty((N, Ho, Wo, cp), dtype=torch.float16, device=x4.device)
        tok = L.TIMER.start(f"conv N{N} {H}x{W} c4->{self.cout} k{self.kh}x{self.kw} s{self.stride} stem") if L.TIMER.enabled else None
        L.check(L.load().vsr_conv2d_stem_f16(L.dptr(x4, torch.float16), L.dptr(self.w, torch.float16), L.optr(self.b),
                                             L.dptr(out, torch.float16), out.shape[3], out_coff, N, H, W, Ho, Wo, self.cout,
                                             self.cout_pad, self.kh, self.kw, self.stride, self.pad, self.pad, self.act,
                                             L.cf(self.slope), L.stream()), "conv2d_stem_f16")
        L.TIMER.stop(tok)
        if L.ROUTES.enabled:
            L.ROUTES.note(f"conv N{N} {H}x{W} c4->{self.cout} k{self.kh}x{self.kw} s{self.stride} stem")
        return out


class HDeconv4s2:

    def __init__(self, weight, bias, act=ACT_NONE, slope=0.1, cin_pad=None):
        w = weight.detach().float()
        self.cout = w.shape[1]
        self.phases = []
        kmap = {0: (3, 1), 1: (2, 0)}
        for py in (0, 1):
            for px in (0, 1):
                wk = w[:, :, list(kmap[py]), :][:, :, :, list(kmap[px])]
                c = HConv(wk.permute(1, 0, 2, 3), bias, stride=1, pad=0, act=act, slope=slope, cin_pad=cin_pad)
                c.pad_y, c.pad_x = (1 if py == 0 else 0), (1 if px == 0 else 0)
                c.oy, c.ox = (2, py), (2, px)
                self.phases.append(c)

    def __call__(self, x, out=None, out_coff=0, in_coff=0):
        N, H, W, in_ld = x.shape
        if out is None:
            cp = pad32(out_coff + self.cout)
            out = cached_zeros(self, "out", (N, 2 * H, 2 * W, cp), x.device)
        c0 = self.phases[0]
        tok = L.TIMER.start(f"deconv4s2 N{N} {H}x{W} c{c0.cin_pad}->{self.cout}") if L.TIMER.enabled else None
        wp = (ctypes.c_void_p * 4)(*[c.w.data_ptr() for c in self.phases])
        L.check(L.load().vsr_deconv4s2_nhwc_f16(
            L.dptr(x, torch.float16), in_ld, in_coff, wp, L.optr(c0.b), L.dptr(out, torch.float16), out.shape[3], out_coff, N, H, W,
            c0.cin_pad, self.cout, c0.cout_pad, c0.act, L.cf(c0.slope), L.dptr(_splitk_ws(x.device)), ctypes.c_size_t(_WS_BYTES),
            L.stream()), "deconv4s2_nhwc_f16")
        L.TIMER.stop(tok)
        if L.ROUTES.enabled:
            L.ROUTES.note(f"deconv4s2 N{N} {H}x{W} c{c0.cin_pad}->{self.cout}")
        return out


class HHourglassFront:

    def __init__(self, stem: "HConvStem", one: "HConv"):
        if (stem.kh, stem.kw, stem.stride, stem.pad, stem.cout, stem.cout_pad, stem.act) != (7, 7, 1, 3, 128, 128, ACT_RELU):
            raise ValueError("HHourglassFront: the stem is Conv2d(3, 128, 7, 1, 3) + ReLU")
        if (one.kh, one.kw, one.stride, one.cin_pad, one.act) != (1, 1, 1, 128, ACT_RELU) or one.cout % 8 or one.cout_pad > 256:
            raise ValueError("HHourglassFront: the second stage is a 1x1 convolution + ReLU over the stem's 128 channels")
        self.stem, self.one = stem, one

    def __call__(self, x4, out2, pooled=None, stem_out=None):
        N, H, W, c4 = x4.shape
        assert c4 == 4 and x4.dtype == torch.float16 and out2.shape[:3] == (N, H, W)
        tok = L.TIMER.start(f"hg_front N{N} {H}x{W} c4->128->{self.one.cout}") if L.TIMER.enabled else None
        L.check(L.load().vsr_hg_front_f16(
            L.dptr(x4, torch.float16), L.dptr(self.stem.w, torch.float16), L.optr(self.stem.b), L.dptr(self.one.w, torch.float16), L.optr(self.one.b),
            self.one.cout, self.one.cout_pad, L.optr(stem_out, torch.float16), stem_out.shape[3] if stem_out is not None else 0,
            L.optr(pooled, torch.float16), L.dptr(out2, torch.float16), out2.shape[3], N, H, W, L.stream()), "hg_front")
        L.TIMER.stop(tok)
        if L.ROUTES.enabled:
            L.ROUTES.note(f"hg_front N{N} {H}x{W} c4->128->{self.one.cout}")
        return out2


class HFlowHead:

    def __init__(self, pred_weight, pred_bias, up_weight=None, up_bias=None, cin_pad=None):
        w = pred_weight.detach().float()
        cout, cin, kh, kw = w.shape
        if (cout, kh, kw) != (2, 3, 3):
            raise ValueError("HFlowHead: predict_flow is Conv2d(cin, 2, 3, 1, 1)")
        dev = w.device
        self.cin_pad = cin_pad or pad32(cin)
        wp = torch.zeros((self.cin_pad // 32, 32, 32), dtype=torch.float32, device=dev)
        wfull = torch.zeros((2, self.cin_pad, 3, 3), dtype=torch.float32, device=dev)
        wfull[:, :cin] = w
        wp[:, :18] = wfull.view(2, self.cin_pad // 32, 32, 9).permute(1, 3, 0, 2).reshape(self.cin_pad // 32, 18, 32)
        self.w = wp.to(torch.float16).contiguous()
        self.b = pred_bias.detach().float().contiguous() if pred_bias is not None else None
        self.up_w = self.up_b = None
        if up_weight is not None:
            if tuple(up_weight.shape) != (2, 2, 4, 4):
                raise ValueError("HFlowHead: the flow upsampling is ConvTranspose2d(2, 2, 4, 2, 1)")
            self.up_w = up_weight.detach().to(torch.float16).float().contiguous()
            self.up_b = up_bias.detach().float().contiguous() if up_bias is not None else None

    def __call__(self, x, up_out=None, up_coff=0, in_coff=0):
        N, H, W, in_ld = x.shape
        flow = cached_zeros(self, "flow", (N, H, W, 32), x.device)
        if (self.up_w is None) != (up_out is None):
            raise ValueError("HFlowHead: `up_out` goes with an upsampling weight")
        tok = L.TIMER.start(f"flow_head N{N} {H}x{W} c{self.cin_pad}") if L.TIMER.enabled else None
        L.check(L.load().vsr_flow_head_f16(
            L.dptr(x, torch.float16), in_ld, in_coff, self.cin_pad, L.dptr(self.w, torch.float16), L.optr(self.b), L.dptr(flow, torch.float16), 32, 0,
            L.optr(self.up_w), L.optr(self.up_b), L.optr(up_out, torch.float16), up_out.shape[3] if up_out is not None else 0, up_coff,
            N, H, W, L.stream()), "flow_head")
        L.TIMER.stop(tok)
        if L.ROUTES.enabled:
            L.ROUTES.note(f"flow_head N{N} {H}x{W} c{self.cin_pad}{' +up' if up_out is not None else ''}")
        return flow


def pool2x2(x, coff, c, mode):
    N, H, W, ld = x.shape
    ho, wo = ((H + 1) // 2, (W + 1) // 2) if mode == 2 else (H // 2, W // 2)
    out = torch.empty((N, ho, wo, c), dtype=torch.float16, device=x.device)
    L.check(L.load().vsr_pool2x2_nhwc_f16(L.dptr(x, torch.float16), ld, coff, L.dptr(out, torch.float16), N, H, W, c, mode, L.stream()),
            "pool2x2")
    return out


class SegMap:

    def __init__(self, segs):
        self.segs = list(segs)
        self.shape = self.segs[0][0].shape

    @property
    def device(self):
        return self.segs[0][0].device

    def record_stream(self, stream):
        for t, _ in self.segs:
            t.record_stream(stream)


def _seg_args(t, coff, c):
    segs = t.segs if isinstance(t, SegMap) else [(t, coff)]
    n = len(segs)
    vp, ip = ctypes.c_void_p * n, ctypes.c_int * n
    for tt, _ in segs:
        if tt.dtype != torch.float16 or not tt.is_contiguous():
            raise L.VsrHipError("resize_add: segments must be dense float16 tensors")
    return vp(*[tt.data_ptr() for tt, _ in segs]), ip(*[tt.shape[3] for tt, _ in segs]), ip(*[co for _, co in segs]), n


def resize_add(a, a_coff, c, out_hw, b=None, b_coff=0, up2=False, b_up2=False):
    N, Ha, Wa, a_ld = a.shape
    H, W = out_hw
    out = torch.empty((N, H, W, c), dtype=torch.float16, device=a.device)
    ap, al, ac, an = _seg_args(a, a_coff, c)
    bp, bl, bc, bn = _seg_args(b, b_coff, c) if b is not None else (None, None, None, 0)
    L.check(L.load().vsr_resize_add_segs_nhwc_f16(ap, al, ac, an, Ha, Wa, 1 if up2 else 0, bp, bl, bc, bn, 1 if b_up2 else 0,
                                                  L.dptr(out, torch.float16), N, H, W, c, L.stream()), "resize_add_segs")
    return out
```

### video_super_resolution_amd/trunk_exec.py

```python
from __future__ import annotations

import ctypes
import os

import torch
import torch.nn as nn
import torch.nn.functional as F

from . import _lib as L
from . import ops
from .depth import HOURGLASS
from .igemm import (ACT_LEAKY, ACT_NONE, ACT_RELU, HConv, HConvPairS2, HConvStem, HDeconv4s2, HFlowHead, HHourglassFront, SegMap, cached_zeros,
                    pad32, pool2x2, resize_add, to_nhwc_half)


def _fold(conv: nn.Conv2d, bn):
    w = conv.weight.detach().float()
    b = conv.bias.detach().float() if conv.bias is not None else torch.zeros(w.shape[0], device=w.device)
    if bn is not None:
        scale = torch.rsqrt(bn.running_var.float() + bn.eps)
        if bn.affine:
            scale = scale * bn.weight.detach().float()
        shift = -bn.running_mean.float() * scale
        if bn.affine:
            shift = shift + bn.bias.detach().float()
        w = w * scale.view(-1, 1, 1, 1)
        b = b * scale + shift
    return w, b


def _nchw(x):
    return x.permute(0, 3, 1, 2)


def _nhwc(x):
    return x.permute(0, 2, 3, 1).contiguous()


class _Inception:

    def __init__(self, mod):
        b0 = mod[0]
        w0, bb0 = _fold(b0[0], b0[1])
        ws, bs, self.kconvs = [], [], []
        mids, outs = [], []
        for j in (1, 2, 3):
            br = mod[j]
            w1, b1 = _fold(br[0], br[1])
            ws.append(w1)
            bs.append(b1)
            mids.append(w1.shape[0])
            wk, bk = _fold(br[3], br[4])
            outs.append(wk.shape[0])
            self.kconvs.append((wk, bk, br[3].kernel_size[0]))
        self.M = sum(mids)
        self.o0 = w0.shape[0]
        self.ctot = self.o0 + sum(outs)
        self.width = pad32(self.M + self.ctot)
        self.first = HConv(torch.cat(ws + [w0], 0), torch.cat(bs + [bb0], 0), act=ACT_RELU)
        packed = []
        moff, ooff = 0, self.M + self.o0
        for (wk, bk, k), mid, o in zip(self.kconvs, mids, outs):
            packed.append((HConv(wk, bk, pad=(k - 1) // 2, act=ACT_RELU), moff, ooff))
            moff += mid
            ooff += o
        self.kconvs = packed
        self.cin = w0.shape[1]

    dense_thin = os.environ.get("VSR_DENSE_THIN", "1") != "0"

    def branches(self, buf):
        if self.dense_thin and all(conv.cout == 16 for conv, _, _ in self.kconvs) and self.o0 == 16:
            N, H, W, _ = buf.shape
            outs = torch.empty((len(self.kconvs), N, H, W, 16), dtype=torch.float16, device=buf.device)
            for j, (conv, moff, _) in enumerate(self.kconvs):
                conv(buf, out=outs[j], out_coff=0, in_coff=moff)
            return SegMap([(buf, self.M)] + [(outs[j], 0) for j in range(len(self.kconvs))]), 0, self.ctot
        for conv, moff, ooff in self.kconvs:
            conv(buf, out=buf, out_coff=ooff, in_coff=moff)
        return buf, self.M, self.ctot

    fused_small = os.environ.get("VSR_HG_INCEPTION", "1") != "0"
    FUSED_SIGS = {(32, (3, 5, 7), 32, 32), (32, (3, 5, 7), 64, 64), (64, (3, 7, 11), 64, 64), (64, (3, 7, 11), 32, 32), (64, (3, 5, 7), 32, 32)}
    FUSED_SMALL_PIXELS = 67 * 120
    FUSED_MAX_PIXELS = 135 * 240
    FUSED_SIGS_TO_MAX = {(128, 32, (3, 5, 7), 64, 64)}

    @staticmethod
    def fused_rule(sig, H, W):
        cin, mid, ks, cout, o0 = sig
        if cin not in (128, 256) or (mid, ks, cout, o0) not in _Inception.FUSED_SIGS or H <= 0 or W <= 0:
            return False
        return H * W <= _Inception.FUSED_SMALL_PIXELS or (H * W <= _Inception.FUSED_MAX_PIXELS and tuple(sig) in _Inception.FUSED_SIGS_TO_MAX)

    def signature(self):
        mids = {conv.cin_pad for conv, _, _ in self.kconvs}
        outs = {conv.cout for conv, _, _ in self.kconvs}
        if len(mids) != 1 or len(outs) != 1 or self.M != 3 * min(mids):
            return None
        return self.cin, min(mids), tuple(conv.kh for conv, _, _ in self.kconvs), min(outs), self.o0

    def fused(self, x, in_coff):
        N, H, W, in_ld = x.shape
        cin, mid, ks, cout, o0 = self.signature()
        out = torch.empty((N, H, W, self.ctot), dtype=torch.float16, device=x.device)
        lib = L.load_hgi()
        args = []
        for conv, _, _ in self.kconvs:
            args += [L.dptr(conv.w, torch.float16), L.dptr(conv.b), conv.kh]
        L.check(lib.vsr_hgi_inception_f16(L.dptr(x, torch.float16), in_ld, in_coff, cin, L.dptr(self.first.w, torch.float16), L.dptr(self.first.b),
                                          self.first.cout_pad, mid, o0, *args, cout, L.dptr(out, torch.float16), self.ctot, N, H, W, L.stream()),
                "hgi_inception", lib=lib)
        if L.ROUTES.enabled:
            L.ROUTES.note_as(f"inception N{N} {H}x{W} c{cin}->{self.ctot} mid{mid}", "hg_inception<%d,%d,%d>" % ks)
        return out, 0, self.ctot

    def __call__(self, x, in_coff):
        N, H, W, _ = x.shape
        if self.fused_small:
            sig = self.signature()
            if sig is not None and self.ctot % 32 == 0 and self.fused_rule(sig, H, W):
                return self.fused(x, in_coff)
        buf = torch.empty((N, H, W, self.width), dtype=torch.float16, device=x.device)
        if self.width != self.M + self.ctot:
            buf[..., self.M + self.ctot:] = 0
        self.first(x, out=buf, out_coff=0, in_coff=in_coff)
        return self.branches(buf)


class HourglassExec:
    fused_front = os.environ.get("VSR_HG_FRONT", "1") != "0"

    def __init__(self, netg: nn.Sequential):
        self.prog = self._build(HOURGLASS, netg)
        self.front = self._match_front(self.prog)

    @staticmethod
    def _match_front(prog):
        try:
            items = prog[1]
            stem, lvl = items[0], items[1]
            fan = lvl[1][0]
            arm_a, arm_b = fan[1]
            ok = (stem[0] == "stem" and stem[2] == 128 and lvl[0] == "S" and lvl[1][1] == "+" and len(lvl[1]) == 2 and fan[0] == "M" and
                  arm_a[0] == "S" and arm_a[1][0] == "max" and arm_b[0] == "S" and len(arm_b[1]) == 1 and arm_b[1][0][0] == "I" and
                  arm_b[1][0][1].cin == 128)
            return HHourglassFront(stem[1], arm_b[1][0][1].first) if ok else None
        except (IndexError, TypeError, ValueError, AttributeError):
            return None

    def _build(self, node, mod):
        if isinstance(node, str):
            return node
        tag = node[0]
        if tag == "S":
            items, children = [], list(mod)
            i = 0
            while i < len(node[1]):
                ch = node[1][i]
                if isinstance(ch, tuple) and ch[0] == "conv":
                    bn = children[i + 1] if i + 1 < len(children) and isinstance(children[i + 1], nn.BatchNorm2d) else None
                    j = i + (2 if bn is not None else 1)
                    relu = j < len(children) and isinstance(children[j], nn.ReLU)
                    w, b = _fold(children[i], bn)
                    if w.shape[1] <= 4 and w.shape[3] <= 8:
                        items.append(("stem", HConvStem(w, b, pad=ch[4], act=ACT_RELU if relu else ACT_NONE), ch[2]))
                    else:
                        items.append(("conv", HConv(w, b, pad=ch[4], act=ACT_RELU if relu else ACT_NONE), ch[2]))
                    i = j + (1 if relu else 0)
                    continue
                items.append(self._build(ch, children[i]))
                i += 1
            return ("S", items)
        if tag == "M":
            return ("M", [self._build(c, m) for c, m in zip(node[1], mod)])
        if tag == "I":
            return ("I", _Inception(mod))
        raise ValueError(node)

    def _side(self, dev, level):
        if L.serial_streams.on:
            return torch.cuda.current_stream(dev)
        key = (dev.type, dev.index)
        if getattr(self, "_side_key", None) != key:
            self._side_streams, self._side_key = {}, key
        if level not in self._side_streams:
            self._side_streams[level] = torch.cuda.Stream(device=dev)
        return self._side_streams[level]

    def _fan_out(self, subs, x, coff, c, level):
        if len(subs) != 2 or not self.concurrent:
            return [self._run(sub, x, coff, c, level + 1) for sub in subs]
        cur = torch.cuda.current_stream(x.device)
        side = self._side(x.device, level)
        side.wait_stream(cur)
        with torch.cuda.stream(side):
            first = self._run(subs[0], x, coff, c, level + 1)
            first[0].record_stream(cur)
        x.record_stream(side)
        second = self._run(subs[1], x, coff, c, level + 1)
        cur.wait_stream(side)
        return [first, second]

    concurrent = os.environ.get("VSR_HOURGLASS_STREAMS", "0") == "1"
    defer_up = True

    def _run(self, node, x, coff, c, level=0):
        if node == "max" or node == "avg":
            return pool2x2(x, coff, c, 0 if node == "max" else 1), 0, c
        if node == "up":
            return resize_add(x, coff, c, (2 * x.shape[1], 2 * x.shape[2])), 0, c
        tag = node[0]
        if tag == "conv":
            if node[2] == 1:
                N, H, W, _ = x.shape
                Ho, Wo = node[1].out_hw(H, W)
                out = node[1](x, in_coff=coff, out=torch.empty((N, Ho, Wo, 1), dtype=torch.float16, device=x.device))
            else:
                out = node[1](x, in_coff=coff)
            return out, 0, node[2]
        if tag == "stem":
            return node[1](x), 0, node[2]
        if tag == "I":
            buf, m, ctot = node[1](x, coff)
            return buf, m, ctot
        if tag == "S":
            items = node[1]
            for i, ch in enumerate(items):
                if ch == "+":
                    a, ca, na = x[0][:3]
                    b, cb, nb = x[1][:3]
                    a_up, b_up = len(x[0]) > 3, len(x[1]) > 3
                    out_hw = (b.shape[1] << b_up, b.shape[2] << b_up)
                    x, coff, c = resize_add(a, ca, nb, out_hw, b, cb, up2=a_up, b_up2=b_up), 0, nb
                elif isinstance(ch, tuple) and ch[0] == "M":
                    x = self._fan_out(ch[1], x, coff, c, level)
                elif ch == "up" and i == len(items) - 1 and self.defer_up:
                    return x, coff, c, "up2"
                else:
                    x, coff, c = self._run(ch, x, coff, c, level)
            return x, coff, c
        raise ValueError(node)

    @L.on_device
    @torch.no_grad()
    def __call__(self, frames_nhwc3: torch.Tensor) -> torch.Tensor:
        k, h, w, _ = frames_nhwc3.shape
        stem_first = self.prog[0] == "S" and isinstance(self.prog[1][0], tuple) and self.prog[1][0][0] == "stem"
        x = cached_zeros(self, "in", (k, h, w, 4 if stem_first else 32), frames_nhwc3.device)
        x[..., :3] = frames_nhwc3
        if self.front is not None and self.fused_front and h >= 2 and w >= 2:
            out, coff, c = self._run_fused_front(x)
        else:
            out, coff, c = self._run(self.prog, x, 0, 32)
        return out[..., coff:coff + 1].permute(0, 3, 1, 2).float()

    def _run_fused_front(self, x4):
        k, h, w, _ = x4.shape
        items = self.prog[1]
        arm_a, arm_b = items[1][1][0][1]
        inc = arm_b[1][0][1]
        buf = torch.empty((k, h, w, inc.width), dtype=torch.float16, device=x4.device)
        if inc.width != inc.M + inc.ctot:
            buf[..., inc.M + inc.ctot:] = 0
        pooled = torch.empty((k, h // 2, w // 2, 128), dtype=torch.float16, device=x4.device)
        self.front(x4, buf, pooled)
        a = self._run(("S", arm_a[1][1:]), pooled, 0, 128, 1)
        x, coff, c = self._run(("S", ["+"]), [a, inc.branches(buf)], 0, 0)
        return self._run(("S", items[2:]), x, coff, c)


def _cv(seq, stride=1, act=ACT_LEAKY, cin_pad=None):
    conv = seq[0] if isinstance(seq, nn.Sequential) else seq
    k = conv.kernel_size[0]
    return HConv(conv.weight, conv.bias, stride=conv.stride[0], pad=(k - 1) // 2, act=act, slope=0.1, cin_pad=cin_pad)


class _Refine:
    fused_heads = os.environ.get("VSR_FLOW_HEADS", "1") != "0"

    def __init__(self, net, with_inter: bool):
        self.with_inter = with_inter
        self.pred6 = _cv(net.predict_flow6, act=ACT_NONE)
        self.levels = []
        prev_pred = net.predict_flow6
        for lvl, cin_cat in ((5, 1026), (4, 770), (3, 386), (2, 194)):
            dec = getattr(net, f"deconv{lvl}")[0]
            up = getattr(net, f"upsampled_flow{lvl + 1}_to_{lvl}")
            item = dict(deconv=HDeconv4s2(dec.weight, dec.bias, act=ACT_LEAKY),
                        upflow=HDeconv4s2(up.weight, up.bias, act=ACT_NONE),
                        cat=pad32(cin_cat), dec_c=dec.weight.shape[1])
            pred = getattr(net, f"predict_flow{lvl}")
            if with_inter:
                item["inter"] = _cv(getattr(net, f"inter_conv{lvl}"), act=ACT_NONE, cin_pad=pad32(cin_cat))
                item["pred"] = _cv(pred, act=ACT_NONE)
            else:
                item["pred"] = _cv(pred, act=ACT_NONE, cin_pad=pad32(cin_cat))
            item["head_in"] = HFlowHead(prev_pred.weight, prev_pred.bias, up.weight, up.bias,
                                        cin_pad=None if (with_inter or lvl == 5) else self.levels[-1]["cat"])
            prev_pred = pred
            self.levels.append(item)
        self.head_last = HFlowHead(prev_pred.weight, prev_pred.bias, cin_pad=None if with_inter else self.levels[-1]["cat"])

    def alloc_cat(self, idx, N, H, W, dev):
        return cached_zeros(self, f"cat{idx}", (N, H, W, self.levels[idx]["cat"]), dev)

    def __call__(self, c6, cats, enc_c):
        if not self.fused_heads:
            flow = self.pred6(c6)
            src = c6
            for i, lv in enumerate(self.levels):
                cat = cats[i]
                lv["deconv"](src, out=cat, out_coff=enc_c[i])
                lv["upflow"](flow, out=cat, out_coff=enc_c[i] + lv["dec_c"])
                flow = lv["pred"](lv["inter"](cat)) if self.with_inter else lv["pred"](cat)
                src = cat
            return flow
        src = head_src = c6
        for i, lv in enumerate(self.levels):
            cat = cats[i]
            lv["deconv"](src, out=cat, out_coff=enc_c[i])
            lv["head_in"](head_src, up_out=cat, up_coff=enc_c[i] + lv["dec_c"])
            src = cat
            head_src = lv["inter"](cat) if self.with_inter else cat
        return self.head_last(head_src)


class _FlowNetSExec:
    def __init__(self, net, cin):
        c1 = net.conv1[0] if isinstance(net.conv1, nn.Sequential) else net.conv1
        self.conv1 = HConvPairS2(c1.weight, c1.bias, pad=(c1.kernel_size[0] - 1) // 2, act=ACT_LEAKY, slope=0.1) \
            if cin <= 16 and c1.stride[0] == 2 else _cv(net.conv1, cin_pad=pad32(cin))
        self.pair_input = isinstance(self.conv1, HConvPairS2)
        self.names = ["conv2", "conv3", "conv3_1", "conv4", "conv4_1", "conv5", "conv5_1", "conv6", "conv6_1"]
        self.convs = {n: _cv(getattr(net, n)) for n in self.names}
        self.refine = _Refine(net, with_inter=False)

    def __call__(self, x):
        N, H, W, _ = x.shape
        dev = x.device
        c1 = self.conv1(x)
        h2, w2 = H // 4, W // 4
        cats = [self.refine.alloc_cat(i, N, H >> (5 - i), W >> (5 - i), dev) for i in range(4)]
        self.convs["conv2"](c1, out=cats[3], out_coff=0)
        self.convs["conv3_1"](self.convs["conv3"](cats[3]), out=cats[2], out_coff=0)
        self.convs["conv4_1"](self.convs["conv4"](cats[2]), out=cats[1], out_coff=0)
        self.convs["conv5_1"](self.convs["conv5"](cats[1]), out=cats[0], out_coff=0)
        c6 = self.convs["conv6_1"](self.convs["conv6"](cats[0]))
        return self.refine(c6, cats, [512, 512, 256, 128])


class _FlowNetCExec:
    def __init__(self, net):
        c1 = net.conv1[0] if isinstance(net.conv1, nn.Sequential) else net.conv1
        self.conv1 = HConvStem(c1.weight, c1.bias, stride=c1.stride[0], pad=(c1.kernel_size[0] - 1) // 2, act=ACT_LEAKY, slope=0.1)
        self.conv2, self.conv3 = _cv(net.conv2), _cv(net.conv3)
        self.redir = _cv(net.conv_redir)
        self.conv3_1 = _cv(net.conv3_1, cin_pad=pad32(473))
        self.names = ["conv4", "conv4_1", "conv5", "conv5_1", "conv6", "conv6_1"]
        self.convs = {n: _cv(getattr(net, n)) for n in self.names}
        self.refine = _Refine(net, with_inter=False)

    def __call__(self, x6, both=None):
        B, H, W, _ = x6.shape
        dev = x6.device
        if both is None:
            both = cached_zeros(self, "both", (2 * B, H, W, 4), dev)
            both[:B, ..., :3] = x6[..., 0:3]
            both[B:, ..., :3] = x6[..., 3:6]
        c2 = self.conv2(self.conv1(both))
        c3 = self.conv3(c2)
        a3, b3 = c3[:B], c3[B:]
        h8, w8 = H // 8, W // 8
        cat31 = cached_zeros(self, "cat31", (B, h8, w8, pad32(473)), dev)
        self.redir(a3, out=cat31, out_coff=0)
        L.check(L.load().vsr_flownetc_corr_nhwc_f16(L.dptr(a3, torch.float16), L.dptr(b3, torch.float16), L.dptr(cat31, torch.float16),
                                                    cat31.shape[3], 32, B, h8, w8, c3.shape[3], L.stream()), "flownetc_corr")
        cats = [self.refine.alloc_cat(i, B, H >> (5 - i), W >> (5 - i), dev) for i in range(4)]
        cats[3][..., :128] = c2[:B]
        self.conv3_1(cat31, out=cats[2], out_coff=0)
        self.convs["conv4_1"](self.convs["conv4"](cats[2]), out=cats[1], out_coff=0)
        self.convs["conv5_1"](self.convs["conv5"](cats[1]), out=cats[0], out_coff=0)
        c6 = self.convs["conv6_1"](self.convs["conv6"](cats[0]))
        return self.refine(c6, cats, [512, 512, 256, 128])


class _FlowNetSDExec:
    def __init__(self, net):
        self.conv0 = _cv(net.conv0, cin_pad=32)
        self.names = ["conv1", "conv1_1", "conv2", "conv2_1", "conv3", "conv3_1", "conv4", "conv4_1", "conv5", "conv5_1",
                      "conv6", "conv6_1"]
        self.convs = {n: _cv(getattr(net, n)) for n in self.names}
        self.refine = _Refine(net, with_inter=True)

    def __call__(self, x6):
        N, H, W, _ = x6.shape
        dev = x6.device
        c = self.convs
        c0 = self.conv0(x6)
        c1 = c["conv1_1"](c["conv1"](c0))
        cats = [self.refine.alloc_cat(i, N, H >> (5 - i), W >> (5 - i), dev) for i in range(4)]
        c["conv2_1"](c["conv2"](c1), out=cats[3], out_coff=0)
        c["conv3_1"](c["conv3"](cats[3]), out=cats[2], out_coff=0)
        c["conv4_1"](c["conv4"](cats[2]), out=cats[1], out_coff=0)
        c["conv5_1"](c["conv5"](cats[1]), out=cats[0], out_coff=0)
        c6 = c["conv6_1"](c["conv6"](cats[0]))
        return self.refine(c6, cats, [512, 512, 256, 128])
# ... 211 lines not shown
```

Before: 45.36.

## Fuse hourglass resize-add sums into the following conv's input load

Adds a new HIP side library with sum+conv kernels (3x3 and streaming 1x1 MFMA) that read the two hourglass addends, optionally 2x-upsampled, and add them while loading conv input. The executor now defers each resize_add as a pending sum and lets an eligible consumer conv take it directly. Otherwise the sum is resolved as before. This removes the write and re-read of the summed intermediate map and one kernel launch per fused site, at the cost of extra address math and gather loads inside the conv. Eligibility rules restrict fusion to large maps and certain channel counts.

```diff
diff --git a/__graft_entry__.py b/__graft_entry__.py
--- a/__graft_entry__.py
+++ b/__graft_entry__.py
@@ -73,6 +73,9 @@
     cellmissing = [s for s in _lib.declared_symbols(cell=True) if not hasattr(_lib.load_cell(), s)]
     if cellmissing:
         raise RuntimeError(f"libvsr_hip_cell.so lacks {cellmissing}")
+    hgsmissing = [s for s in _lib.declared_symbols(hgs=True) if not hasattr(_lib.load_hgs(), s)]
+    if hgsmissing:
+        raise RuntimeError(f"libvsr_hip_hgs.so lacks {hgsmissing}")
 
 
 def smoke() -> None:
diff --git a/include/vsr_hip_hgs.h b/include/vsr_hip_hgs.h
--- /dev/null
+++ b/include/vsr_hip_hgs.h
@@ -0,0 +1,32 @@
+#ifndef VSR_HIP_HGS_H
+#define VSR_HIP_HGS_H
+
+#include "vsr_hip.h"
+
+#ifdef __cplusplus
+extern "C" {
+#endif
+
+#define VSR_HGS_ABI_VERSION 1
+
+#define VSR_HGS_CONV3X3 3
+#define VSR_HGS_CONV1X1 1
+
+int vsr_hgs_abi_version(void);
+const char* vsr_hgs_last_error(void);
+
+int vsr_hgs_supported(int kind, int H, int W, int cin, int cout);
+
+int vsr_hgs_sum_conv3x3_f16(const void* const* a_ptrs, const int* a_lds, const int* a_coffs, int a_nseg, int Ha, int Wa, int up2,
+                            const void* const* b_ptrs, const int* b_lds, const int* b_coffs, int b_nseg, int b_up2, const void* w_packed,
+                            const float* bias, void* out, int out_ld, int out_coff, int N, int H, int W, int cin, int cout, int cout_pad, int act,
+                            float slope, vsr_stream_t stream);
+int vsr_hgs_sum_conv1x1_f16(const void* const* a_ptrs, const int* a_lds, const int* a_coffs, int a_nseg, int Ha, int Wa, int up2,
+                            const void* const* b_ptrs, const int* b_lds, const int* b_coffs, int b_nseg, int b_up2, const void* w_packed,
+                            const float* bias, void* out, int out_ld, int out_coff, int N, int H, int W, int cin, int cout, int cout_pad, int act,
+                            float slope, vsr_stream_t stream);
+
+#ifdef __cplusplus
+}
+#endif
+#endif
diff --git a/video_super_resolution_amd/_lib.py b/video_super_resolution_amd/_lib.py
--- a/video_super_resolution_amd/_lib.py
+++ b/video_super_resolution_amd/_lib.py
@@ -28,13 +28,13 @@
          "scene": _side("scene", "vsr_scene", 1, False), "hgi": _side("hgi", "vsr_hgi", 1, False),
          "msssim": _side("msssim", "vsr_msssim", 1, False), "pix": _side("pix", "vsr_pix", 1, False),
          "patch": _side("patch", "vsr_patch", 1, False), "deint": _side("deint", "vsr_deint", 1, False),
-         "cell": _side("cell", "vsr_cell", 1, False)}
+         "cell": _side("cell", "vsr_cell", 1, False), "hgs": _side("hgs", "vsr_hgs", 1, False)}
 (GLIB_PATH, GHEADER_PATH), (S3LIB_PATH, S3HEADER_PATH), (S3TLIB_PATH, S3THEADER_PATH), (S3PLIB_PATH, S3PHEADER_PATH), \
     (S3FLIB_PATH, S3FHEADER_PATH), (YUVLIB_PATH, YUVHEADER_PATH), (METRICLIB_PATH, METRICHEADER_PATH), (OPTLIB_PATH, OPTHEADER_PATH), \
     (LOSSLIB_PATH, LOSSHEADER_PATH), (RESIZELIB_PATH, RESIZEHEADER_PATH), (WARPLIB_PATH, WARPHEADER_PATH), (SCENELIB_PATH, SCENEHEADER_PATH), \
     (HGILIB_PATH, HGIHEADER_PATH), (MSSSIMLIB_PATH, MSSSIMHEADER_PATH), (PIXLIB_PATH, PIXHEADER_PATH), (PATCHLIB_PATH, PATCHHEADER_PATH), \
-    (DEINTLIB_PATH, DEINTHEADER_PATH), (CELLLIB_PATH, CELLHEADER_PATH) = (row[:2] for row in _SIDE.values())
-_gradlib = _s3lib = _s3tlib = _s3plib = _s3flib = _yuvlib = _metriclib = _optlib = _losslib = _resizelib = _warplib = _scenelib = _hgilib = _msssimlib = _pixlib = _patchlib = _deintlib = _celllib = None
+    (DEINTLIB_PATH, DEINTHEADER_PATH), (CELLLIB_PATH, CELLHEADER_PATH), (HGSLIB_PATH, HGSHEADER_PATH) = (row[:2] for row in _SIDE.values())
+_gradlib = _s3lib = _s3tlib = _s3plib = _s3flib = _yuvlib = _metriclib = _optlib = _losslib = _resizelib = _warplib = _scenelib = _hgilib = _msssimlib = _pixlib = _patchlib = _deintlib = _celllib = _hgslib = None
 _use_x = os.environ.get("VSR_USE_XCHECK", "0") == "1" or bool(os.environ.get("VSR_TUNING", "").strip())
 
 
@@ -53,10 +53,10 @@
 def declared_symbols(xcheck: bool = False, grad: bool = False, s3: bool = False, s3t: bool = False, s3p: bool = False, s3f: bool = False,
                      yuv: bool = False, metric: bool = False, opt: bool = False, loss: bool = False, resize: bool = False,
                      warp: bool = False, scene: bool = False, hgi: bool = False, msssim: bool = False, pix: bool = False,
-                     patch: bool = False, deint: bool = False, cell: bool = False) -> list:
+                     patch: bool = False, deint: bool = False, cell: bool = False, hgs: bool = False) -> list:
     side = [name for name, on in (("grad", grad), ("s3", s3), ("s3t", s3t), ("s3p", s3p), ("s3f", s3f), ("yuv", yuv), ("metric", metric),
                                   ("opt", opt), ("loss", loss), ("resize", resize), ("warp", warp), ("scene", scene), ("hgi", hgi),
-                                  ("msssim", msssim), ("pix", pix), ("patch", patch), ("deint", deint), ("cell", cell)) if on]
+                                  ("msssim", msssim), ("pix", pix), ("patch", patch), ("deint", deint), ("cell", cell), ("hgs", hgs)) if on]
     with open(_SIDE[side[-1]][1] if side else XHEADER_PATH if xcheck else HEADER_PATH) as f:
         text = re.sub(r"/\*.*?\*/", "", f.read(), flags=re.S)
     return sorted(set(re.findall(r"\b(vsr_[a-z0-9_]+)\s*\(", text)))
@@ -229,6 +229,15 @@
     return lib
 
 
+def load_hgs() -> ctypes.CDLL:
+    lib = _load_side("hgs")
+    seg = [ctypes.c_void_p] * 3 + [ctypes.c_int]
+    for fn in (lib.vsr_hgs_sum_conv3x3_f16, lib.vsr_hgs_sum_conv1x1_f16):
+        fn.argtypes = seg + [ctypes.c_int] * 3 + seg + [ctypes.c_int] + [ctypes.c_void_p] * 3 + [ctypes.c_int] * 9 + [ctypes.c_float, ctypes.c_void_p]
+    lib.vsr_hgs_supported.argtypes = [ctypes.c_int] * 5
+    return lib
+
+
 def load() -> ctypes.CDLL:
     global _lib
     if _use_x:
diff --git a/video_super_resolution_amd/csrc/conv1x1_stream.h b/video_super_resolution_amd/csrc/conv1x1_stream.h
--- /dev/null
+++ b/video_super_resolution_amd/csrc/conv1x1_stream.h
@@ -0,0 +1,157 @@
+#pragma once
+#include <cstdint>
+
+#include "conv_common.h"
+#include "conv_sum_load.h"
+
+namespace vsrc {
+
+constexpr int C1_MAX_CHUNKS = 8;
+template <int NCH, class LD>
+__global__ void __launch_bounds__(512) k_conv1x1_stream(const typename LD::Params p) {
+    constexpr bool LATE_A = LD::SUM && NCH > 4;
+    constexpr int NS = LD::SUM && !LATE_A ? NCH : 1;
+    extern __shared__ __attribute__((aligned(16))) unsigned char wsm[];
+    const int tid = threadIdx.x, lane = tid & 63, wv = tid >> 6;
+    const int l15 = lane & 15, g = lane >> 4;
+    const long long M = (long long)p.N * p.Ho * p.Wo;
+    const int rows = NCH * p.cout_pad;
+    for (int q = tid; q < rows * 4; q += 512)
+        *reinterpret_cast<uint4*>(wsm + sw_off(q >> 2, q & 3)) = *reinterpret_cast<const uint4*>(p.wpk + (size_t)q * 8);
+    float* const bsm = reinterpret_cast<float*>(wsm + (size_t)rows * 64);
+    for (int q = tid; q < p.cout_pad; q += 512) bsm[q] = (p.bias && q < p.cout) ? p.bias[q] : 0.0f;
+    __syncthreads();
+    const int ntile = min(p.cout_pad >> 4, 2 * ((p.cout + 31) >> 5));
+    const long long nblk = (M + 255) / 256;
+    h8 bf[NCH][2], nx[NCH][2];
+    h8 na[NS][2];
+    [[maybe_unused]] auto pixels = [&](long long m, unsigned& ia, unsigned& ib) __attribute__((always_inline)) {
+        if constexpr (LD::SUM) {
+            const unsigned mm = (unsigned)(m < M ? m : M - 1);
+            const unsigned row = mm / (unsigned)p.W, x = mm - row * (unsigned)p.W;
+            const unsigned n = row / (unsigned)p.H, y = row - n * (unsigned)p.H;
+            vsrc::sum_pixels(p, (int)n, (int)y, (int)x, ia, ib);
+        }
+    };
+    auto fetch = [&](long long blk, h8 (&dst)[NCH][2]) __attribute__((always_inline)) {
+#pragma unroll
+        for (int nt = 0; nt < 2; ++nt) {
+            const long long m = blk * 256 + 32 * wv + 16 * nt + l15;
+            if constexpr (!LD::SUM) {
+                const _Float16* src = p.in + (size_t)(m < M ? m : M - 1) * p.in_ld + p.in_coff + 8 * g;
+#pragma unroll
+                for (int c = 0; c < NCH; ++c) dst[c][nt] = *reinterpret_cast<const h8*>(src + 32 * c);
+            } else {
+                unsigned ia, ib;
+                pixels(m, ia, ib);
+#pragma unroll
+                for (int c = 0; c < NCH; ++c) {
+                    int ald, bld;
+                    const _Float16* const ap = vsrc::sum_seg_piece(p.a, 32 * c + 8 * g, ald);
+                    const _Float16* const bp = vsrc::sum_seg_piece(p.b, 32 * c + 8 * g, bld);
+                    if constexpr (!LATE_A) na[c][nt] = *reinterpret_cast<const h8*>(ap + (size_t)ia * (unsigned)ald);
+                    dst[c][nt] = *reinterpret_cast<const h8*>(bp + (size_t)ib * (unsigned)bld);
+                }
+            }
+        }
+    };
+    if ((long long)blockIdx.x < nblk) fetch(blockIdx.x, nx);
+    for (long long blk = blockIdx.x; blk < nblk; blk += gridDim.x) {
+        const long long mbase = blk * 256 + 32 * wv;
+#pragma unroll
+        for (int c = 0; c < NCH; ++c)
+#pragma unroll
+            for (int nt = 0; nt < 2; ++nt) {
+                if constexpr (!LD::SUM) bf[c][nt] = nx[c][nt];
+                else if constexpr (!LATE_A) bf[c][nt] = na[c][nt] + nx[c][nt];
+            }
+        if constexpr (LATE_A) {
+#pragma unroll
+            for (int nt = 0; nt < 2; ++nt) {
+                unsigned ia, ib;
+                pixels(mbase + 16 * nt + l15, ia, ib);
+#pragma unroll
+                for (int c = 0; c < NCH; ++c) {
+                    int ald;
+                    const _Float16* const ap = vsrc::sum_seg_piece(p.a, 32 * c + 8 * g, ald);
+                    bf[c][nt] = *reinterpret_cast<const h8*>(ap + (size_t)ia * (unsigned)ald) + nx[c][nt];
+                }
+            }
+        }
+        if (blk + gridDim.x < nblk) fetch(blk + gridDim.x, nx);
+        const float nslope = p.act == 1 ? 0.0f : (p.act == 2 ? p.slope : 1.0f);
+        const bool vec_ok = (p.out_coff & 7) == 0 && (p.out_ld & 7) == 0;
+        int t = 0;
+        for (; t + 1 < ntile; t += 2) {
+            const int rowA = 16 * t + 8 * (l15 >> 2) + (l15 & 3);
+            h8 a0[NCH], a1[NCH];
+#pragma unroll
+            for (int c = 0; c < NCH; ++c) {
+                a0[c] = *reinterpret_cast<const h8*>(wsm + sw_off(c * p.cout_pad + rowA, g));
+                a1[c] = *reinterpret_cast<const h8*>(wsm + sw_off(c * p.cout_pad + rowA + 4, g));
+            }
+            const int c0 = 16 * t + 8 * g;
+            const f4 b0 = *reinterpret_cast<const f4*>(bsm + c0), b1 = *reinterpret_cast<const f4*>(bsm + c0 + 4);
+            f4 acc[2][2];
+#pragma unroll
+            for (int nt = 0; nt < 2; ++nt) { acc[0][nt] = b0; acc[1][nt] = b1; }
+#pragma unroll
+            for (int c = 0; c < NCH; ++c)
+#pragma unroll
+                for (int nt = 0; nt < 2; ++nt) {
+                    acc[0][nt] = __builtin_amdgcn_mfma_f32_16x16x32_f16(a0[c], bf[c][nt], acc[0][nt], 0, 0, 0);
+                    acc[1][nt] = __builtin_amdgcn_mfma_f32_16x16x32_f16(a1[c], bf[c][nt], acc[1][nt], 0, 0, 0);
+                }
+            const bool full = vec_ok && c0 + 8 <= p.cout;
+#pragma unroll
+            for (int nt = 0; nt < 2; ++nt) {
+                const long long m = mbase + 16 * nt + l15;
+                float v[8];
+#pragma unroll
+                for (int r = 0; r < 8; ++r) {
+                    const float x = acc[r >> 2][nt][r & 3];
+                    v[r] = fmaxf(x, 0.0f) + nslope * fminf(x, 0.0f);
+                }
+                _Float16* dst = p.out + (size_t)(m < M ? m : 0) * p.out_ld + p.out_coff + c0;
+                if (m < M && full) {
+                    *reinterpret_cast<h8*>(dst) = h8{(_Float16)v[0], (_Float16)v[1], (_Float16)v[2], (_Float16)v[3],
+                                                     (_Float16)v[4], (_Float16)v[5], (_Float16)v[6], (_Float16)v[7]};
+                } else if (m < M) {
+#pragma unroll
+                    for (int r = 0; r < 8; ++r)
+                        if (c0 + r < p.cout) dst[r] = (_Float16)v[r];
+                }
+            }
+        }
+        if (t < ntile) {
+            h8 a0[NCH];
+#pragma unroll
+            for (int c = 0; c < NCH; ++c) a0[c] = *reinterpret_cast<const h8*>(wsm + sw_off(c * p.cout_pad + 16 * t + l15, g));
+            const int c0 = 16 * t + 4 * g;
+            const f4 b0 = *reinterpret_cast<const f4*>(bsm + c0);
+            f4 acc[2] = {b0, b0};
+#pragma unroll
+            for (int c = 0; c < NCH; ++c)
+#pragma unroll
+                for (int nt = 0; nt < 2; ++nt) acc[nt] = __builtin_amdgcn_mfma_f32_16x16x32_f16(a0[c], bf[c][nt], acc[nt], 0, 0, 0);
+            const bool full = (p.out_coff & 3) == 0 && (p.out_ld & 3) == 0 && c0 + 4 <= p.cout;
+#pragma unroll
+            for (int nt = 0; nt < 2; ++nt) {
+                const long long m = mbase + 16 * nt + l15;
+                float v[4];
+#pragma unroll
+                for (int r = 0; r < 4; ++r) v[r] = fmaxf(acc[nt][r], 0.0f) + nslope * fminf(acc[nt][r], 0.0f);
+                _Float16* dst = p.out + (size_t)(m < M ? m : 0) * p.out_ld + p.out_coff + c0;
+                if (m < M && full) {
+                    *reinterpret_cast<h4*>(dst) = h4{(_Float16)v[0], (_Float16)v[1], (_Float16)v[2], (_Float16)v[3]};
+                } else if (m < M) {
+#pragma unroll
+                    for (int r = 0; r < 4; ++r)
+                        if (c0 + r < p.cout) dst[r] = (_Float16)v[r];
+                }
+            }
+        }
+    }
+}
+
+}
diff --git a/video_super_resolution_amd/csrc/conv_hg_sums.hip b/video_super_resolution_amd/csrc/conv_hg_sums.hip
--- /dev/null
+++ b/video_super_resolution_amd/csrc/conv_hg_sums.hip
@@ -0,0 +1,120 @@
+#include <cstdint>
+
+#include "conv1x1_stream.h"
+#include "conv_patch_pf.h"
+
+#include "../../include/vsr_hip_hgs.h"
+
+namespace {
+
+using vsrc::SumConvP;
+using vsrc::SumLoad;
+using vsrc::SumSeg;
+
+uintptr_t addr(const void* q) { return reinterpret_cast<uintptr_t>(q); }
+
+int cout_pad_of(int cout) { return cout <= 16 ? 16 : cout <= 32 ? 32 : (cout + 63) / 64 * 64; }
+
+int fill_seg(SumSeg& s, const char* what, const char* who, const void* const* ptrs, const int* lds, const int* coffs, int nseg, int cin) {
+    VSR_REQUIRE(ptrs && lds && coffs, "%s: null pointer (segment lists of %s)", what, who);
+    VSR_REQUIRE(nseg >= 1 && nseg <= 4 && cin % nseg == 0 && ((cin / nseg) & 7) == 0, "%s: %d segments of %s for %d channels (1 to 4 of equal width, a multiple of 8)",
+                what, nseg, who, cin);
+    s.seg_c = cin / nseg;
+    for (int i = 0; i < 4; ++i) {
+        const int j = i < nseg ? i : 0;
+        VSR_REQUIRE(ptrs[j], "%s: null pointer (segment %d of %s)", what, j, who);
+        VSR_REQUIRE((addr(ptrs[j]) & 15) == 0 && lds[j] > 0 && (lds[j] & 7) == 0 && coffs[j] >= 0 && (coffs[j] & 7) == 0 && coffs[j] + s.seg_c <= lds[j],
+                    "%s: misaligned segment %d of %s (16-byte pointer, ld and coff multiples of 8, coff + %d <= ld)", what, j, who, s.seg_c);
+        s.ptr[i] = (const _Float16*)ptrs[j]; s.ld[i] = lds[j]; s.coff[i] = coffs[j];
+    }
+    return VSR_OK;
+}
+
+int make_sum(SumConvP& p, const char* what, int kh, const void* const* a_ptrs, const int* a_lds, const int* a_coffs, int a_nseg, int Ha, int Wa, int up2,
+             const void* const* b_ptrs, const int* b_lds, const int* b_coffs, int b_nseg, int b_up2, const void* w_packed, const float* bias, void* out,
+             int out_ld, int out_coff, int N, int H, int W, int cin, int cout, int cout_pad, int act, float slope) {
+    VSR_REQUIRE(w_packed && out, "%s: null pointer", what);
+    VSR_REQUIRE(N > 0 && H > 0 && W > 0 && Ha > 0 && Wa > 0 && N <= 65535, "%s: bad shape (N %d, map of %d x %d from %d x %d)", what, N, H, W, Ha, Wa);
+    VSR_REQUIRE((long long)N * H * W < (1ll << 31) && (long long)N * Ha * Wa < (1ll << 31), "%s: bad shape (a map of 2^31 pixels or more)", what);
+    VSR_REQUIRE(cin >= 32 && cin <= 256 && (cin & 31) == 0, "%s: bad shape (cin %d: a multiple of 32 up to 256)", what, cin);
+    VSR_REQUIRE((up2 == 0 || up2 == 1) && (b_up2 == 0 || b_up2 == 1), "%s: up2 flags", what);
+    VSR_REQUIRE(b_up2 == 0 || ((H & 1) == 0 && (W & 1) == 0), "%s: up2 flags (an upsampled addend needs an even output size, not %d x %d)", what, H, W);
+    VSR_REQUIRE(act >= 0 && act <= 2, "%s: bad shape (act %d)", what, act);
+    VSR_REQUIRE(cout >= 1 && cout <= cout_pad && (cout_pad & 15) == 0, "%s: bad shape (cout %d, cout_pad %d)", what, cout, cout_pad);
+    VSR_REQUIRE(((addr(w_packed) | addr(out)) & 15) == 0 && (addr(bias) & 3) == 0, "%s: w_packed and out must be 16-byte aligned", what);
+    VSR_REQUIRE(out_ld > 0 && out_coff >= 0 && out_coff + cout <= out_ld, "%s: the output slice [%d, %d) leaves its row of %d", what, out_coff, out_coff + cout,
+                out_ld);
+    p = SumConvP{};
+    int rc = fill_seg(p.a, what, "a", a_ptrs, a_lds, a_coffs, a_nseg, cin);
+    if (rc) return rc;
+    rc = fill_seg(p.b, what, "b", b_ptrs, b_lds, b_coffs, b_nseg, cin);
+    if (rc) return rc;
+    p.Ha = Ha; p.Wa = Wa; p.up2 = up2; p.b_up2 = b_up2;
+    p.in = nullptr; p.in_ld = cin; p.in_coff = 0;
+    p.wpk = (const _Float16*)w_packed; p.bias = bias; p.out = (_Float16*)out; p.out_ld = out_ld; p.out_coff = out_coff;
+    p.N = N; p.H = H; p.W = W; p.cin = cin; p.Ho = H; p.Wo = W; p.cout = cout; p.cout_pad = cout_pad;
+    p.kh = p.kw = kh; p.stride = p.stride_x = 1; p.pad_y = p.pad_x = (kh - 1) / 2;
+    p.outH = H; p.outW = W; p.oy_mul = p.ox_mul = 1; p.oy_off = p.ox_off = 0;
+    p.act = act; p.slope = slope; p.ws = nullptr; p.splits = 1; p.nphase = 0;
+    return VSR_OK;
+}
+
+}
+
+extern "C" {
+
+int vsr_hgs_abi_version(void) { return VSR_HGS_ABI_VERSION; }
+const char* vsr_hgs_last_error(void) { return vsr::err_buf(); }
+
+int vsr_hgs_supported(int kind, int H, int W, int cin, int cout) {
+    if (H <= 0 || W <= 0 || cin < 32 || cin > 256 || (cin & 31) || cout < 1) return 0;
+    const long long px = (long long)H * W;
+    if (kind == VSR_HGS_CONV3X3)
+        return cout <= 16 && H >= 12 && W >= 16 && px >= 8192 && (unsigned long long)(3 + 16) * W * cin * 2 < (1ull << 31);
+    if (kind == VSR_HGS_CONV1X1) {
+        const int cp = cout_pad_of(cout);
+        return px >= 65536 && cp > 64 && (size_t)(cin >> 5) * cp * 64 <= 128 * 1024;
+    }
+    return 0;
+}
+
+int vsr_hgs_sum_conv3x3_f16(const void* const* a_ptrs, const int* a_lds, const int* a_coffs, int a_nseg, int Ha, int Wa, int up2,
+                            const void* const* b_ptrs, const int* b_lds, const int* b_coffs, int b_nseg, int b_up2, const void* w_packed,
+                            const float* bias, void* out, int out_ld, int out_coff, int N, int H, int W, int cin, int cout, int cout_pad, int act,
+                            float slope, vsr_stream_t stream) {
+    static const char* const what = "hgs_sum_conv3x3";
+    SumConvP p;
+    const int rc = make_sum(p, what, 3, a_ptrs, a_lds, a_coffs, a_nseg, Ha, Wa, up2, b_ptrs, b_lds, b_coffs, b_nseg, b_up2, w_packed, bias, out, out_ld,
+                            out_coff, N, H, W, cin, cout, cout_pad, act, slope);
+    if (rc) return rc;
+    VSR_REQUIRE(cout <= 16 && cout_pad == 16, "%s: bad shape (cout %d, cout_pad %d: up to 16 in one tile of 16)", what, cout, cout_pad);
+    const int lrc = vsrc::launch_pf<3, 1, 2, SumLoad>(p, N, vsr::S(stream), what);
+    return lrc ? lrc : vsr::launched(what);
+}
+
+int vsr_hgs_sum_conv1x1_f16(const void* const* a_ptrs, const int* a_lds, const int* a_coffs, int a_nseg, int Ha, int Wa, int up2,
+                            const void* const* b_ptrs, const int* b_lds, const int* b_coffs, int b_nseg, int b_up2, const void* w_packed,
+                            const float* bias, void* out, int out_ld, int out_coff, int N, int H, int W, int cin, int cout, int cout_pad, int act,
+                            float slope, vsr_stream_t stream) {
+    static const char* const what = "hgs_sum_conv1x1";
+    typedef void (*kernel_t)(const SumConvP);
+    SumConvP p;
+    const int rc = make_sum(p, what, 1, a_ptrs, a_lds, a_coffs, a_nseg, Ha, Wa, up2, b_ptrs, b_lds, b_coffs, b_nseg, b_up2, w_packed, bias, out, out_ld,
+                            out_coff, N, H, W, cin, cout, cout_pad, act, slope);
+    if (rc) return rc;
+    const size_t w_bytes = (size_t)(cin >> 5) * cout_pad * 64;
+    VSR_REQUIRE(cout_pad > 64 && w_bytes <= 128 * 1024, "%s: bad shape (cout_pad %d above 64, packed weights of %zu B within 128 KiB)", what, cout_pad, w_bytes);
+    static const kernel_t k1[vsrc::C1_MAX_CHUNKS] = {vsrc::k_conv1x1_stream<1, SumLoad>, vsrc::k_conv1x1_stream<2, SumLoad>, vsrc::k_conv1x1_stream<3, SumLoad>,
+                                                     vsrc::k_conv1x1_stream<4, SumLoad>, vsrc::k_conv1x1_stream<5, SumLoad>, vsrc::k_conv1x1_stream<6, SumLoad>,
+                                                     vsrc::k_conv1x1_stream<7, SumLoad>, vsrc::k_conv1x1_stream<8, SumLoad>};
+    const kernel_t k = k1[(cin >> 5) - 1];
+    const size_t k_lds = w_bytes + (size_t)cout_pad * 4;
+    if (k_lds > 48 * 1024 && hipFuncSetAttribute(reinterpret_cast<const void*>(k), hipFuncAttributeMaxDynamicSharedMemorySize, (int)k_lds) != hipSuccess)
+        return vsr::fail(VSR_E_LAUNCH, "%s: cannot reserve %zu bytes of LDS", what, k_lds);
+    const int per_cu = (int)((160 * 1024) / k_lds) < 2 ? 1 : 2;
+    const long long nblk = ((long long)N * H * W + 255) / 256;
+    hipLaunchKernelGGL(k, dim3((unsigned)(nblk < 256LL * per_cu ? nblk : 256LL * per_cu)), dim3(512), k_lds, vsr::S(stream), p);
+    return vsr::launched(what);
+}
+
+}
diff --git a/video_super_resolution_amd/csrc/conv_igemm.hip b/video_super_resolution_amd/csrc/conv_igemm.hip
--- a/video_super_resolution_amd/csrc/conv_igemm.hip
+++ b/video_super_resolution_amd/csrc/conv_igemm.hip
@@ -1,6 +1,7 @@
 #include "conv_common.h"
 #include "conv_kwalk.h"
 #include "conv_patch.h"
+#include "conv1x1_stream.h"
 
 namespace {
 
@@ -368,113 +369,8 @@
 }
 
 
-constexpr int C1_MAX_CHUNKS = 8;
-template <int NCH>
-__global__ void __launch_bounds__(512) k_conv1x1_stream(const ConvP p) {
-    extern __shared__ __attribute__((aligned(16))) unsigned char wsm[];
-    const int tid = threadIdx.x, lane = tid & 63, wv = tid >> 6;
-    const int l15 = lane & 15, g = lane >> 4;
-    const long long M = (long long)p.N * p.Ho * p.Wo;
-    const int rows = NCH * p.cout_pad;
-    for (int q = tid; q < rows * 4; q += 512)
-        *reinterpret_cast<uint4*>(wsm + sw_off(q >> 2, q & 3)) = *reinterpret_cast<const uint4*>(p.wpk + (size_t)q * 8);
-    float* const bsm = reinterpret_cast<float*>(wsm + (size_t)rows * 64);
-    for (int q = tid; q < p.cout_pad; q += 512) bsm[q] = (p.bias && q < p.cout) ? p.bias[q] : 0.0f;
-    __syncthreads();
-    const int ntile = min(p.cout_pad >> 4, 2 * ((p.cout + 31) >> 5));
-    const long long nblk = (M + 255) / 256;
-    h8 bf[NCH][2], nx[NCH][2];
-    auto fetch = [&](long long blk, h8 (&dst)[NCH][2]) __attribute__((always_inline)) {
-#pragma unroll
-        for (int nt = 0; nt < 2; ++nt) {
-            const long long m = blk * 256 + 32 * wv + 16 * nt + l15;
-            const _Float16* src = p.in + (size_t)(m < M ? m : M - 1) * p.in_ld + p.in_coff + 8 * g;
-#pragma unroll
-            for (int c = 0; c < NCH; ++c) dst[c][nt] = *reinterpret_cast<const h8*>(src + 32 * c);
-        }
-    };
-    if ((long long)blockIdx.x < nblk) fetch(blockIdx.x, nx);
-    for (long long blk = blockIdx.x; blk < nblk; blk += gridDim.x) {
-        const long long mbase = blk * 256 + 32 * wv;
-#pragma unroll
-        for (int c = 0; c < NCH; ++c)
-#pragma unroll
-            for (int nt = 0; nt < 2; ++nt) bf[c][nt] = nx[c][nt];
-        if (blk + gridDim.x < nblk) fetch(blk + gridDim.x, nx);
-        const float nslope = p.act == 1 ? 0.0f : (p.act == 2 ? p.slope : 1.0f);
-        const bool vec_ok = (p.out_coff & 7) == 0 && (p.out_ld & 7) == 0;
-        int t = 0;
-        for (; t + 1 < ntile; t += 2) {
-            const int rowA = 16 * t + 8 * (l15 >> 2) + (l15 & 3);
-            h8 a0[NCH], a1[NCH];
-#pragma unroll
-            for (int c = 0; c < NCH; ++c) {
-                a0[c] = *reinterpret_cast<const h8*>(wsm + sw_off(c * p.cout_pad + rowA, g));
-                a1[c] = *reinterpret_cast<const h8*>(wsm + sw_off(c * p.cout_pad + rowA + 4, g));
-            }
-            const int c0 = 16 * t + 8 * g;
-            const f4 b0 = *reinterpret_cast<const f4*>(bsm + c0), b1 = *reinterpret_cast<const f4*>(bsm + c0 + 4);
-            f4 acc[2][2];
-#pragma unroll
-            for (int nt = 0; nt < 2; ++nt) { acc[0][nt] = b0; acc[1][nt] = b1; }
-#pragma unroll
-            for (int c = 0; c < NCH; ++c)
-#pragma unroll
-                for (int nt = 0; nt < 2; ++nt) {
-                    acc[0][nt] = __builtin_amdgcn_mfma_f32_16x16x32_f16(a0[c], bf[c][nt], acc[0][nt], 0, 0, 0);
-                    acc[1][nt] = __builtin_amdgcn_mfma_f32_16x16x32_f16(a1[c], bf[c][nt], acc[1][nt], 0, 0, 0);
-                }
-            const bool full = vec_ok && c0 + 8 <= p.cout;
-#pragma unroll
-            for (int nt = 0; nt < 2; ++nt) {
-                const long long m = mbase + 16 * nt + l15;
-                float v[8];
-#pragma unroll
-                for (int r = 0; r < 8; ++r) {
-                    const float x = acc[r >> 2][nt][r & 3];
-                    v[r] = fmaxf(x, 0.0f) + nslope * fminf(x, 0.0f);
-                }
-                _Float16* dst = p.out + (size_t)(m < M ? m : 0) * p.out_ld + p.out_coff + c0;
-                if (m < M && full) {
-                    *reinterpret_cast<h8*>(dst) = h8{(_Float16)v[0], (_Float16)v[1], (_Float16)v[2], (_Float16)v[3],
-                                                     (_Float16)v[4], (_Float16)v[5], (_Float16)v[6], (_Float16)v[7]};
-                } else if (m < M) {
-#pragma unroll
-                    for (int r = 0; r < 8; ++r)
-                        if (c0 + r < p.cout) dst[r] = (_Float16)v[r];
-                }
-            }
-        }
-        if (t < ntile) {
-            h8 a0[NCH];
-#pragma unroll
-            for (int c = 0; c < NCH; ++c) a0[c] = *reinterpret_cast<const h8*>(wsm + sw_off(c * p.cout_pad + 16 * t + l15, g));
-            const int c0 = 16 * t + 4 * g;
-            const f4 b0 = *reinterpret_cast<const f4*>(bsm + c0);
-            f4 acc[2] = {b0, b0};
-#pragma unroll
-            for (int c = 0; c < NCH; ++c)
-#pragma unroll
-                for (int nt = 0; nt < 2; ++nt) acc[nt] = __builtin_amdgcn_mfma_f32_16x16x32_f16(a0[c], bf[c][nt], acc[nt], 0, 0, 0);
-            const bool full = (p.out_coff & 3) == 0 && (p.out_ld & 3) == 0 && c0 + 4 <= p.cout;
-#pragma unroll
-            for (int nt = 0; nt < 2; ++nt) {
-                const long long m = mbase + 16 * nt + l15;
-                float v[4];
-#pragma unroll
-                for (int r = 0; r < 4; ++r) v[r] = fmaxf(acc[nt][r], 0.0f) + nslope * fminf(acc[nt][r], 0.0f);
-                _Float16* dst = p.out + (size_t)(m < M ? m : 0) * p.out_ld + p.out_coff + c0;
-                if (m < M && full) {
-                    *reinterpret_cast<h4*>(dst) = h4{(_Float16)v[0], (_Float16)v[1], (_Float16)v[2], (_Float16)v[3]};
-                } else if (m < M) {
-#pragma unroll
-                    for (int r = 0; r < 4; ++r)
-                        if (c0 + r < p.cout) dst[r] = (_Float16)v[r];
-                }
-            }
-        }
-    }
-}
+using vsrc::C1_MAX_CHUNKS;
+using vsrc::PlainLoad;
 
 #if VSR_X
 constexpr int C1T_SLOT = 32 * 256;
@@ -1328,8 +1224,8 @@
         break;
     }
     case Kind::conv1x1_stream: {
-        static const conv_kernel_t k1[C1_MAX_CHUNKS] = {k_conv1x1_stream<1>, k_conv1x1_stream<2>, k_conv1x1_stream<3>, k_conv1x1_stream<4>,
-                                                        k_conv1x1_stream<5>, k_conv1x1_stream<6>, k_conv1x1_stream<7>, k_conv1x1_stream<8>};
+        static const conv_kernel_t k1[C1_MAX_CHUNKS] = {vsrc::k_conv1x1_stream<1, PlainLoad>, vsrc::k_conv1x1_stream<2, PlainLoad>, vsrc::k_conv1x1_stream<3, PlainLoad>, vsrc::k_conv1x1_stream<4, PlainLoad>,
+                                                        vsrc::k_conv1x1_stream<5, PlainLoad>, vsrc::k_conv1x1_stream<6, PlainLoad>, vsrc::k_conv1x1_stream<7, PlainLoad>, vsrc::k_conv1x1_stream<8, PlainLoad>};
         const conv_kernel_t k = k1[(p.cin >> 5) - 1];
         const size_t k_lds = (size_t)(p.cin >> 5) * p.cout_pad * 64 + (size_t)p.cout_pad * 4;
         if (k_lds > 48 * 1024 &&
diff --git a/video_super_resolution_amd/csrc/conv_patch_pf.h b/video_super_resolution_amd/csrc/conv_patch_pf.h
--- /dev/null
+++ b/video_super_resolution_amd/csrc/conv_patch_pf.h
@@ -0,0 +1,191 @@
+#pragma once
+#include "conv_patch.h"
+#include "conv_sum_load.h"
+
+namespace vsrc {
+
+template <int KH, int MT, int WPS, class LD>
+__global__ void __launch_bounds__(256, WPS) k_conv_patch_pf(const typename LD::Params p, int tiles_x, int tiles_y, int nwork) {
+    typedef vsrc::u4 u4v;
+    typedef vsrc::P8Geom<KH, MT> G;
+    constexpr int PH = G::PH, PW = G::PW, NPC = G::NPC, NWC = G::NWC, WTAP = G::WTAP;
+    constexpr int NPA = LD::SUM ? NPC : 1;
+    extern __shared__ __attribute__((aligned(16))) unsigned char psm[];
+    unsigned char* const patch = psm;
+    unsigned char* const wts = psm + G::WOFF;
+    const int tid = threadIdx.x, lane = tid & 63, wv = __builtin_amdgcn_readfirstlane(tid >> 6);
+    const int l15 = lane & 15, g = lane >> 4;
+    const int nchunk = p.cin >> 5, nblk = p.cout_pad / (16 * MT);
+    const int ry0 = P8_R * (wv >> 1), cx0 = 16 * (wv & 1);
+
+    const __amdgpu_buffer_rsrc_t w_rsrc = __builtin_amdgcn_make_buffer_rsrc(
+        const_cast<_Float16*>(p.wpk), 0, (int)((size_t)KH * KH * nchunk * p.cout_pad * 64), 0x00020000);
+    int wdst[NWC];
+    unsigned wsrc[NWC];
+#pragma unroll
+    for (int j = 0; j < NWC; ++j) {
+        const int q = tid + 256 * j;
+        const int row = q >> 2, slot = q & 3, tap = row / (16 * MT), r = row - tap * (16 * MT);
+        const bool in = q * 16 < G::WBYTES;
+        wdst[j] = in ? tap * WTAP + sw_off(r, slot) : -1;
+        wsrc[j] = in ? (unsigned)(((size_t)tap * nchunk * p.cout_pad + r) * 64 + slot * 16) : 0xFFFFFFFFu;
+    }
+
+    f4 acc[P8_R][MT];
+#pragma unroll
+    for (int r = 0; r < P8_R; ++r)
+#pragma unroll
+        for (int mt = 0; mt < MT; ++mt) acc[r][mt] = f4{0.0f, 0.0f, 0.0f, 0.0f};
+
+    u4v pf[NPC + NWC];
+    unsigned poff[NPC];
+    int pdst[NPC];
+    u4v pa[NPA];
+    unsigned aidx[NPA], bidx[NPA];
+    struct Item { int n, oy0, ox0, co0, by; };
+    auto decode = [&](int w) {
+        Item it;
+        const int blk = w % nblk, t = w / nblk;
+        const int tx = t % tiles_x, t2 = t / tiles_x, ty = t2 % tiles_y;
+        it.n = t2 / tiles_y;
+        it.oy0 = ty * P8_H; it.ox0 = tx * P8_W; it.co0 = blk * 16 * MT;
+        const int iy0 = it.oy0 - p.pad_y;
+        it.by = iy0 > 0 ? iy0 : 0;
+        return it;
+    };
+    [[maybe_unused]] auto sum_pieces = [&](const Item& it) __attribute__((always_inline)) {
+        if constexpr (LD::SUM) {
+            const int iy0 = it.oy0 - p.pad_y, ix0 = it.ox0 - p.pad_x;
+            const int total = PH * PW * 4;
+            const int c4 = tid & 3;
+            int pix = tid >> 2, py = pix / PW, px = pix - py * PW;
+            const int dpy = 64 / PW, dpx = 64 - dpy * PW;
+#pragma unroll
+            for (int k = 0; k < NPC; ++k) {
+                const int iy = iy0 + py, ix = ix0 + px;
+                const bool in = pix * 4 < total;
+                const bool ok = in && (unsigned)iy < (unsigned)p.H && (unsigned)ix < (unsigned)p.W;
+                aidx[k] = bidx[k] = 0xFFFFFFFFu;
+                if (ok) vsrc::sum_pixels(p, it.n, iy, ix, aidx[k], bidx[k]);
+                pdst[k] = in ? pix * 64 + ((c4 ^ ((px >> 1) & 3)) << 4) : -1;
+                pix += 64; py += dpy; px += dpx;
+                if (px >= PW) { px -= PW; ++py; }
+            }
+        }
+    };
+    auto issue = [&](const Item& it, int ch) __attribute__((always_inline)) {
+        if constexpr (!LD::SUM) {
+            const __amdgpu_buffer_rsrc_t rs = vsrc::patch_rsrc_at(p, it.n, it.by);
+#pragma unroll
+            for (int k = 0; k < NPC; ++k) pf[k] = __builtin_amdgcn_raw_buffer_load_b128(rs, vsrc::cached_piece_off(poff[k], ch), 0, 0);
+        } else {
+            int ald, bld;
+            const _Float16* const ap = vsrc::sum_seg_piece(p.a, 32 * ch + 8 * (tid & 3), ald);
+            const _Float16* const bp = vsrc::sum_seg_piece(p.b, 32 * ch + 8 * (tid & 3), bld);
+#pragma unroll
+            for (int k = 0; k < NPC; ++k) {
+                const bool ok = aidx[k] != 0xFFFFFFFFu;
+                pa[k] = *reinterpret_cast<const u4v*>(ap + (size_t)(ok ? aidx[k] : 0u) * (unsigned)ald);
+                pf[k] = *reinterpret_cast<const u4v*>(bp + (size_t)(ok ? bidx[k] : 0u) * (unsigned)bld);
+            }
+        }
+        const unsigned woff = (unsigned)(((size_t)ch * p.cout_pad + it.co0) * 64);
+#pragma unroll
+        for (int j = 0; j < NWC; ++j)
+            pf[NPC + j] = __builtin_amdgcn_raw_buffer_load_b128(w_rsrc, wsrc[j] == 0xFFFFFFFFu ? 0xFFFFFFFFu : wsrc[j] + woff, 0, 0);
+    };
+    auto commit = [&]() __attribute__((always_inline)) {
+#pragma unroll
+        for (int k = 0; k < NPC; ++k) {
+            if constexpr (!LD::SUM) {
+                if (pdst[k] >= 0) *reinterpret_cast<u4v*>(patch + pdst[k]) = pf[k];
+            } else {
+                h8 s = __builtin_bit_cast(h8, pa[k]) + __builtin_bit_cast(h8, pf[k]);
+                if (aidx[k] == 0xFFFFFFFFu) s = h8{0, 0, 0, 0, 0, 0, 0, 0};
+                if (pdst[k] >= 0) *reinterpret_cast<h8*>(patch + pdst[k]) = s;
+            }
+        }
+#pragma unroll
+        for (int j = 0; j < NWC; ++j)
+            if (wdst[j] >= 0) *reinterpret_cast<u4v*>(wts + wdst[j]) = pf[NPC + j];
+    };
+
+    int w = blockIdx.x;
+    if (w >= nwork) return;
+    Item cur = decode(w);
+    if constexpr (!LD::SUM) vsrc::patch_pieces(p, cur.oy0 - p.pad_y, cur.ox0 - p.pad_x, PH, PW, tid, poff, pdst);
+    else sum_pieces(cur);
+    issue(cur, 0);
+    Item nxt = cur;
+    int ch = 0;
+    while (true) {
+        __syncthreads();
+        commit();
+        __syncthreads();
+        const bool last_chunk = ch + 1 == nchunk;
+        const int w2 = last_chunk ? w + (int)gridDim.x : w;
+        const bool have_next = !last_chunk || w2 < nwork;
+        if (have_next) {
+            if (last_chunk) {
+                nxt = decode(w2);
+                if constexpr (!LD::SUM) vsrc::patch_pieces(p, nxt.oy0 - p.pad_y, nxt.ox0 - p.pad_x, PH, PW, tid, poff, pdst);
+                else sum_pieces(nxt);
+            }
+            issue(nxt, last_chunk ? 0 : ch + 1);
+        }
+#pragma unroll 1
+        for (int kx = 0; kx < KH; ++kx) {
+            h8 A[KH][MT];
+#pragma unroll
+            for (int ky = 0; ky < KH; ++ky)
+#pragma unroll
+                for (int mt = 0; mt < MT; ++mt)
+                    A[ky][mt] = *reinterpret_cast<const h8*>(wts + (ky * KH + kx) * WTAP + sw_off(16 * mt + l15, g));
+            const int px = cx0 + l15 + kx;
+            const unsigned char* src = patch + (ry0 * PW + px) * 64 + ((g ^ ((px >> 1) & 3)) << 4);
+#pragma unroll
+            for (int pr = 0; pr < KH + P8_R - 1; ++pr) {
+                const h8 bf = *reinterpret_cast<const h8*>(src + pr * PW * 64);
+#pragma unroll
+                for (int r = 0; r < P8_R; ++r) {
+                    const int ky = pr - r;
+                    if (ky < 0 || ky >= KH) continue;
+#pragma unroll
+                    for (int mt = 0; mt < MT; ++mt) acc[r][mt] = __builtin_amdgcn_mfma_f32_16x16x32_f16(A[ky][mt], bf, acc[r][mt], 0, 0, 0);
+                }
+            }
+        }
+        if (!last_chunk) { ++ch; continue; }
+        __syncthreads();
+        {
+            const vsrc::WaveOut wo = vsrc::wave_out(p, cur.n, cur.oy0 + ry0, cur.ox0 + cx0);
+            vsrc::patch_epilogue<MT, P8_R>(p, psm + wv * (P8_R * 16 * 32 * MT), cur.co0, lane, [&](int r, int mt) { return acc[r][mt]; },
+                                           [&](int r, int li) { return r < wo.rows_ok && li < wo.cols_ok ? wo.wbase + r * wo.rstride + li * wo.cstride : -1ll; });
+        }
+        if (!have_next) break;
+#pragma unroll
+        for (int r = 0; r < P8_R; ++r)
+#pragma unroll
+            for (int mt = 0; mt < MT; ++mt) acc[r][mt] = f4{0.0f, 0.0f, 0.0f, 0.0f};
+        cur = nxt; w = w2; ch = 0;
+    }
+}
+
+template <int KH, int MT, int WPS, class LD>
+int launch_pf(const typename LD::Params& p, int N, hipStream_t stream, const char* what) {
+    typedef vsrc::P8Geom<KH, MT> G;
+    static unsigned long long raised = 0;
+    if (G::LDS > 64 * 1024) vsr::raise_lds_limit_once(raised, &k_conv_patch_pf<KH, MT, WPS, LD>, 160 * 1024);
+    const int tiles_x = (int)vsr::cdiv(p.Wo, P8_W), tiles_y = (int)vsr::cdiv(p.Ho, P8_H);
+    const long long nwork = (long long)N * tiles_x * tiles_y * (p.cout_pad / (16 * MT));
+    if (nwork >= (1ll << 30)) return vsr::fail(VSR_E_ARG, "%s: %lld work items", what, nwork);
+    int per_cu = (160 * 1024) / G::LDS;
+    if (per_cu > WPS) per_cu = WPS;
+    if (per_cu < 1) per_cu = 1;
+    const long long resident = 256LL * per_cu;
+    const unsigned grid = (unsigned)(nwork < resident ? nwork : resident);
+    hipLaunchKernelGGL((k_conv_patch_pf<KH, MT, WPS, LD>), dim3(grid), dim3(256), G::LDS, stream, p, tiles_x, tiles_y, (int)nwork);
+    return VSR_OK;
+}
+
+}
diff --git a/video_super_resolution_amd/csrc/conv_patch_pf.hip b/video_super_resolution_amd/csrc/conv_patch_pf.hip
--- a/video_super_resolution_amd/csrc/conv_patch_pf.hip
+++ b/video_super_resolution_amd/csrc/conv_patch_pf.hip
@@ -1,157 +1,4 @@
-#include "conv_patch.h"
-
-namespace {
-
-using vsrc::ConvP;
-using vsrc::f4;
-using vsrc::h8;
-using vsrc::P8_H;
-using vsrc::P8_R;
-using vsrc::P8_W;
-using vsrc::sw_off;
-
-typedef vsrc::u4 u4v;
-
-template <int KH, int MT, int WPS>
-__global__ void __launch_bounds__(256, WPS) k_conv_patch_pf(const ConvP p, int tiles_x, int tiles_y, int nwork) {
-    typedef vsrc::P8Geom<KH, MT> G;
-    constexpr int PH = G::PH, PW = G::PW, NPC = G::NPC, NWC = G::NWC, WTAP = G::WTAP;
-    extern __shared__ __attribute__((aligned(16))) unsigned char psm[];
-    unsigned char* const patch = psm;
-    unsigned char* const wts = psm + G::WOFF;
-    const int tid = threadIdx.x, lane = tid & 63, wv = __builtin_amdgcn_readfirstlane(tid >> 6);
-    const int l15 = lane & 15, g = lane >> 4;
-    const int nchunk = p.cin >> 5, nblk = p.cout_pad / (16 * MT);
-    const int ry0 = P8_R * (wv >> 1), cx0 = 16 * (wv & 1);
-
-    const __amdgpu_buffer_rsrc_t w_rsrc = __builtin_amdgcn_make_buffer_rsrc(
-        const_cast<_Float16*>(p.wpk), 0, (int)((size_t)KH * KH * nchunk * p.cout_pad * 64), 0x00020000);
-    int wdst[NWC];
-    unsigned wsrc[NWC];
-#pragma unroll
-    for (int j = 0; j < NWC; ++j) {
-        const int q = tid + 256 * j;
-        const int row = q >> 2, slot = q & 3, tap = row / (16 * MT), r = row - tap * (16 * MT);
-        const bool in = q * 16 < G::WBYTES;
-        wdst[j] = in ? tap * WTAP + sw_off(r, slot) : -1;
-        wsrc[j] = in ? (unsigned)(((size_t)tap * nchunk * p.cout_pad + r) * 64 + slot * 16) : 0xFFFFFFFFu;
-    }
-
-    f4 acc[P8_R][MT];
-#pragma unroll
-    for (int r = 0; r < P8_R; ++r)
-#pragma unroll
-        for (int mt = 0; mt < MT; ++mt) acc[r][mt] = f4{0.0f, 0.0f, 0.0f, 0.0f};
-
-    u4v pf[NPC + NWC];
-    unsigned poff[NPC];
-    int pdst[NPC];
-    struct Item { int n, oy0, ox0, co0, by; };
-    auto decode = [&](int w) {
-        Item it;
-        const int blk = w % nblk, t = w / nblk;
-        const int tx = t % tiles_x, t2 = t / tiles_x, ty = t2 % tiles_y;
-        it.n = t2 / tiles_y;
-        it.oy0 = ty * P8_H; it.ox0 = tx * P8_W; it.co0 = blk * 16 * MT;
-        const int iy0 = it.oy0 - p.pad_y;
-        it.by = iy0 > 0 ? iy0 : 0;
-        return it;
-    };
-    auto issue = [&](const Item& it, int ch) __attribute__((always_inline)) {
-        const __amdgpu_buffer_rsrc_t rs = vsrc::patch_rsrc_at(p, it.n, it.by);
-#pragma unroll
-        for (int k = 0; k < NPC; ++k) pf[k] = __builtin_amdgcn_raw_buffer_load_b128(rs, vsrc::cached_piece_off(poff[k], ch), 0, 0);
-        const unsigned woff = (unsigned)(((size_t)ch * p.cout_pad + it.co0) * 64);
-#pragma unroll
-        for (int j = 0; j < NWC; ++j)
-            pf[NPC + j] = __builtin_amdgcn_raw_buffer_load_b128(w_rsrc, wsrc[j] == 0xFFFFFFFFu ? 0xFFFFFFFFu : wsrc[j] + woff, 0, 0);
-    };
-    auto commit = [&]() __attribute__((always_inline)) {
-#pragma unroll
-        for (int k = 0; k < NPC; ++k)
-            if (pdst[k] >= 0) *reinterpret_cast<u4v*>(patch + pdst[k]) = pf[k];
-#pragma unroll
-        for (int j = 0; j < NWC; ++j)
-            if (wdst[j] >= 0) *reinterpret_cast<u4v*>(wts + wdst[j]) = pf[NPC + j];
-    };
-
-    int w = blockIdx.x;
-    if (w >= nwork) return;
-    Item cur = decode(w);
-    vsrc::patch_pieces(p, cur.oy0 - p.pad_y, cur.ox0 - p.pad_x, PH, PW, tid, poff, pdst);
-    issue(cur, 0);
-    Item nxt = cur;
-    int ch = 0;
-    while (true) {
-        __syncthreads();
-        commit();
-        __syncthreads();
-        const bool last_chunk = ch + 1 == nchunk;
-        const int w2 = last_chunk ? w + (int)gridDim.x : w;
-        const bool have_next = !last_chunk || w2 < nwork;
-        if (have_next) {
-            if (last_chunk) {
-                nxt = decode(w2);
-                vsrc::patch_pieces(p, nxt.oy0 - p.pad_y, nxt.ox0 - p.pad_x, PH, PW, tid, poff, pdst);
-            }
-            issue(nxt, last_chunk ? 0 : ch + 1);
-        }
-#pragma unroll 1
-        for (int kx = 0; kx < KH; ++kx) {
-            h8 A[KH][MT];
-#pragma unroll
-            for (int ky = 0; ky < KH; ++ky)
-#pragma unroll
-                for (int mt = 0; mt < MT; ++mt)
-                    A[ky][mt] = *reinterpret_cast<const h8*>(wts + (ky * KH + kx) * WTAP + sw_off(16 * mt + l15, g));
-            const int px = cx0 + l15 + kx;
-            const unsigned char* src = patch + (ry0 * PW + px) * 64 + ((g ^ ((px >> 1) & 3)) << 4);
-#pragma unroll
-            for (int pr = 0; pr < KH + P8_R - 1; ++pr) {
-                const h8 bf = *reinterpret_cast<const h8*>(src + pr * PW * 64);
-#pragma unroll
-                for (int r = 0; r < P8_R; ++r) {
-                    const int ky = pr - r;
-                    if (ky < 0 || ky >= KH) continue;
-#pragma unroll
-                    for (int mt = 0; mt < MT; ++mt) acc[r][mt] = __builtin_amdgcn_mfma_f32_16x16x32_f16(A[ky][mt], bf, acc[r][mt], 0, 0, 0);
-                }
-            }
-        }
-        if (!last_chunk) { ++ch; continue; }
-        __syncthreads();
-        {
-            const vsrc::WaveOut wo = vsrc::wave_out(p, cur.n, cur.oy0 + ry0, cur.ox0 + cx0);
-            vsrc::patch_epilogue<MT, P8_R>(p, psm + wv * (P8_R * 16 * 32 * MT), cur.co0, lane, [&](int r, int mt) { return acc[r][mt]; },
-                                           [&](int r, int li) { return r < wo.rows_ok && li < wo.cols_ok ? wo.wbase + r * wo.rstride + li * wo.cstride : -1ll; });
-        }
-        if (!have_next) break;
-#pragma unroll
-        for (int r = 0; r < P8_R; ++r)
-#pragma unroll
-            for (int mt = 0; mt < MT; ++mt) acc[r][mt] = f4{0.0f, 0.0f, 0.0f, 0.0f};
-        cur = nxt; w = w2; ch = 0;
-    }
-}
-
-template <int KH, int MT, int WPS>
-int launch_pf(const ConvP& p, int N, hipStream_t stream) {
-    typedef vsrc::P8Geom<KH, MT> G;
-    static unsigned long long raised = 0;
-    if (G::LDS > 64 * 1024) vsr::raise_lds_limit_once(raised, &k_conv_patch_pf<KH, MT, WPS>, 160 * 1024);
-    const int tiles_x = (int)vsr::cdiv(p.Wo, P8_W), tiles_y = (int)vsr::cdiv(p.Ho, P8_H);
-    const long long nwork = (long long)N * tiles_x * tiles_y * (p.cout_pad / (16 * MT));
-    if (nwork >= (1ll << 30)) return vsr::fail(VSR_E_ARG, "conv2d/patch_pf: %lld work items", nwork);
-    int per_cu = (160 * 1024) / G::LDS;
-    if (per_cu > WPS) per_cu = WPS;
-    if (per_cu < 1) per_cu = 1;
-    const long long resident = 256LL * per_cu;
-    const unsigned grid = (unsigned)(nwork < resident ? nwork : resident);
-    hipLaunchKernelGGL((k_conv_patch_pf<KH, MT, WPS>), dim3(grid), dim3(256), G::LDS, stream, p, tiles_x, tiles_y, (int)nwork);
-    return VSR_OK;
-}
-
-}
+#include "conv_patch_pf.h"
 
 namespace vsrc {
 
@@ -159,9 +6,9 @@
 
 int launch_conv_patch_pf(const ConvP& p, int mt, hipStream_t stream) {
     const int N = p.N;
-    if (p.kh == 3 && mt == 1) return launch_pf<3, 1, 3>(p, N, stream);
-    if (p.kh == 3 && mt == 2) return launch_pf<3, 2, 2>(p, N, stream);
-    if (p.kh == 5 && mt == 1) return launch_pf<5, 1, 2>(p, N, stream);
+    if (p.kh == 3 && mt == 1) return launch_pf<3, 1, 3, PlainLoad>(p, N, stream, "conv2d/patch_pf");
+    if (p.kh == 3 && mt == 2) return launch_pf<3, 2, 2, PlainLoad>(p, N, stream, "conv2d/patch_pf");
+    if (p.kh == 5 && mt == 1) return launch_pf<5, 1, 2, PlainLoad>(p, N, stream, "conv2d/patch_pf");
     return vsr::fail(VSR_E_ARG, "conv2d/patch_pf: no build for %dx%d with %d out-channels per workgroup", p.kh, p.kw, 16 * mt);
 }
 
diff --git a/video_super_resolution_amd/csrc/conv_sum_load.h b/video_super_resolution_amd/csrc/conv_sum_load.h
--- /dev/null
+++ b/video_super_resolution_amd/csrc/conv_sum_load.h
@@ -0,0 +1,41 @@
+#pragma once
+#include "conv_common.h"
+
+namespace vsrc {
+
+struct SumSeg {
+    const _Float16* ptr[4];
+    int ld[4], coff[4];
+    int seg_c;
+};
+struct SumConvP : ConvP {
+    SumSeg a, b;
+    int Ha, Wa, up2, b_up2;
+};
+
+struct PlainLoad {
+    typedef ConvP Params;
+    static constexpr bool SUM = false;
+};
+struct SumLoad {
+    typedef SumConvP Params;
+    static constexpr bool SUM = true;
+};
+
+__device__ __forceinline__ int sum_near(int d, int in, int out, int up2) {
+    const int s = in << up2;
+    return min((int)floorf((float)d * ((float)s / (float)out)), s - 1) >> up2;
+}
+__device__ __forceinline__ void sum_pixels(const SumConvP& p, int n, int y, int x, unsigned& ia, unsigned& ib) {
+    ia = (unsigned)((n * p.Ha + sum_near(y, p.Ha, p.H, p.up2)) * p.Wa + sum_near(x, p.Wa, p.W, p.up2));
+    ib = (unsigned)((n * (p.H >> p.b_up2) + (y >> p.b_up2)) * (p.W >> p.b_up2) + (x >> p.b_up2));
+}
+__device__ __forceinline__ const _Float16* sum_seg_piece(const SumSeg& s, int ch, int& ld) {
+    const int i = ch / s.seg_c, c = ch - i * s.seg_c;
+    const _Float16* ptr = i == 0 ? s.ptr[0] : i == 1 ? s.ptr[1] : i == 2 ? s.ptr[2] : s.ptr[3];
+    const int co = i == 0 ? s.coff[0] : i == 1 ? s.coff[1] : i == 2 ? s.coff[2] : s.coff[3];
+    ld = i == 0 ? s.ld[0] : i == 1 ? s.ld[1] : i == 2 ? s.ld[2] : s.ld[3];
+    return ptr + co + c;
+}
+
+}
diff --git a/video_super_resolution_amd/igemm.py b/video_super_resolution_amd/igemm.py
--- a/video_super_resolution_amd/igemm.py
+++ b/video_super_resolution_amd/igemm.py
@@ -309,4 +309,24 @@
     bp, bl, bc, bn = _seg_args(b, b_coff, c) if b is not None else (None, None, None, 0)
     L.check(L.load().vsr_resize_add_segs_nhwc_f16(ap, al, ac, an, Ha, Wa, 1 if up2 else 0, bp, bl, bc, bn, 1 if b_up2 else 0,
                                                   L.dptr(out, torch.float16), N, H, W, c, L.stream()), "resize_add_segs")
+    if L.ROUTES.enabled:
+        L.ROUTES.note_as(f"resize_add N{N} {H}x{W} c{c}", "resize_add_segs")
     return out
+
+
+def sum_conv(kind, conv: HConv, a, a_coff, b, b_coff, c, out_hw, up2, b_up2, out, out_coff=0):
+    N, Ha, Wa, _ = a.shape
+    H, W = out_hw
+    ap, al, ac, an = _seg_args(a, a_coff, c)
+    bp, bl, bc, bn = _seg_args(b, b_coff, c)
+    lib = L.load_hgs()
+    fn, what = (lib.vsr_hgs_sum_conv3x3_f16, "hgs_sum_conv3x3") if kind == 3 else (lib.vsr_hgs_sum_conv1x1_f16, "hgs_sum_conv1x1")
+    label = f"sum+conv N{N} {H}x{W} c{c}->{conv.cout} k{conv.kh}x{conv.kw} s1"
+    tok = L.TIMER.start(label) if L.TIMER.enabled else None
+    L.check(fn(ap, al, ac, an, Ha, Wa, 1 if up2 else 0, bp, bl, bc, bn, 1 if b_up2 else 0, L.dptr(conv.w, torch.float16), L.optr(conv.b),
+               L.dptr(out, torch.float16), out.shape[3], out_coff, N, H, W, c, conv.cout, conv.cout_pad, conv.act, L.cf(conv.slope), L.stream()),
+            what, lib=lib)
+    L.TIMER.stop(tok)
+    if L.ROUTES.enabled:
+        L.ROUTES.note_as(label, "hgs_sum_patch_pf<3,1>" if kind == 3 else "hgs_sum_conv1x1_stream<%d>" % (c // 32))
+    return out
diff --git a/video_super_resolution_amd/trunk_exec.py b/video_super_resolution_amd/trunk_exec.py
--- a/video_super_resolution_amd/trunk_exec.py
+++ b/video_super_resolution_amd/trunk_exec.py
@@ -11,7 +11,7 @@
 from . import ops
 from .depth import HOURGLASS
 from .igemm import (ACT_LEAKY, ACT_NONE, ACT_RELU, HConv, HConvPairS2, HConvStem, HDeconv4s2, HFlowHead, HHourglassFront, SegMap, cached_zeros,
-                    pad32, pool2x2, resize_add, to_nhwc_half)
+                    pad32, pool2x2, resize_add, sum_conv, to_nhwc_half)
 
 
 def _fold(conv: nn.Conv2d, bn):
@@ -35,6 +35,45 @@
 
 def _nhwc(x):
     return x.permute(0, 2, 3, 1).contiguous()
+
+
+SUM_CONV3X3, SUM_CONV1X1 = 3, 1
+
+
+def sum_rule(kind, H, W, cin, cout):
+    if H <= 0 or W <= 0 or cin < 32 or cin > 256 or cin % 32 or cout < 1:
+        return False
+    if kind == SUM_CONV3X3:
+        return cout <= 16 and H >= 12 and W >= 16 and H * W >= 8192 and (3 + 16) * W * cin * 2 < (1 << 31)
+    if kind == SUM_CONV1X1:
+        cout_pad = 16 if cout <= 16 else 32 if cout <= 32 else (cout + 63) // 64 * 64
+        return H * W >= 65536 and cout_pad > 64 and (cin // 32) * cout_pad * 64 <= 128 * 1024
+    return False
+
+
+class _PendingSum:
+
+    def __init__(self, a, ca, b, cb, c, out_hw, a_up, b_up):
+        self.a, self.ca, self.b, self.cb, self.c, self.out_hw, self.a_up, self.b_up = a, ca, b, cb, c, out_hw, a_up, b_up
+        self.shape = (b.shape[0], out_hw[0], out_hw[1], c)
+
+    @property
+    def device(self):
+        return self.b.device
+
+    def takes(self, kind, cout):
+        N, H, W, c = self.shape
+        return kind in HourglassExec.SUM_ROUTES and not L._use_x and sum_rule(kind, H, W, c, cout)
+
+    def resolve(self):
+        return resize_add(self.a, self.ca, self.c, self.out_hw, self.b, self.cb, up2=self.a_up, b_up2=self.b_up)
+
+    def conv(self, kind, hconv, out, out_coff=0):
+        return sum_conv(kind, hconv, self.a, self.ca, self.b, self.cb, self.c, self.out_hw, self.a_up, self.b_up, out, out_coff)
+
+
+def _resolved(x):
+    return x.resolve() if isinstance(x, _PendingSum) else x
 
 
 class _Inception:
@@ -120,11 +159,14 @@
         if self.fused_small:
             sig = self.signature()
             if sig is not None and self.ctot % 32 == 0 and self.fused_rule(sig, H, W):
-                return self.fused(x, in_coff)
+                return self.fused(_resolved(x), in_coff)
         buf = torch.empty((N, H, W, self.width), dtype=torch.float16, device=x.device)
         if self.width != self.M + self.ctot:
             buf[..., self.M + self.ctot:] = 0
-        self.first(x, out=buf, out_coff=0, in_coff=in_coff)
+        if isinstance(x, _PendingSum) and x.c == self.first.cin_pad and x.takes(SUM_CONV1X1, self.first.cout):
+            x.conv(SUM_CONV1X1, self.first, buf)
+        else:
+            self.first(_resolved(x), out=buf, out_coff=0, in_coff=in_coff)
         return self.branches(buf)
 
 
@@ -190,34 +232,49 @@
 
     def _fan_out(self, subs, x, coff, c, level):
         if len(subs) != 2 or not self.concurrent:
-            return [self._run(sub, x, coff, c, level + 1) for sub in subs]
+            return [self._arm(sub, x, coff, c, level + 1) for sub in subs]
         cur = torch.cuda.current_stream(x.device)
         side = self._side(x.device, level)
         side.wait_stream(cur)
         with torch.cuda.stream(side):
-            first = self._run(subs[0], x, coff, c, level + 1)
+            first = self._arm(subs[0], x, coff, c, level + 1)
             first[0].record_stream(cur)
         x.record_stream(side)
-        second = self._run(subs[1], x, coff, c, level + 1)
+        second = self._arm(subs[1], x, coff, c, level + 1)
         cur.wait_stream(side)
         return [first, second]
 
+    def _arm(self, sub, x, coff, c, level):
+        r = self._run(sub, x, coff, c, level)
+        return (_resolved(r[0]),) + tuple(r[1:])
+
+    fused_sums = os.environ.get("VSR_HG_SUMS", "1") != "0"
+    SUM_ROUTES = (SUM_CONV3X3, SUM_CONV1X1)
+
     concurrent = os.environ.get("VSR_HOURGLASS_STREAMS", "0") == "1"
     defer_up = True
 
     def _run(self, node, x, coff, c, level=0):
+        if isinstance(x, _PendingSum) and not (isinstance(node, tuple) and node[0] in ("S", "I", "conv")):
+            x = x.resolve()
         if node == "max" or node == "avg":
             return pool2x2(x, coff, c, 0 if node == "max" else 1), 0, c
         if node == "up":
             return resize_add(x, coff, c, (2 * x.shape[1], 2 * x.shape[2])), 0, c
         tag = node[0]
         if tag == "conv":
+            conv = node[1]
             if node[2] == 1:
                 N, H, W, _ = x.shape
-                Ho, Wo = node[1].out_hw(H, W)
-                out = node[1](x, in_coff=coff, out=torch.empty((N, Ho, Wo, 1), dtype=torch.float16, device=x.device))
+                Ho, Wo = conv.out_hw(H, W)
+                out = torch.empty((N, Ho, Wo, 1), dtype=torch.float16, device=x.device)
+                if isinstance(x, _PendingSum) and (conv.kh, conv.kw, conv.stride, conv.pad_y, conv.pad_x, conv.cin_pad) == (3, 3, 1, 1, 1, x.c) and \
+                        x.takes(SUM_CONV3X3, conv.cout):
+                    x.conv(SUM_CONV3X3, conv, out)
+                else:
+                    conv(_resolved(x), in_coff=coff, out=out)
             else:
-                out = node[1](x, in_coff=coff)
+                out = conv(_resolved(x), in_coff=coff)
             return out, 0, node[2]
         if tag == "stem":
             return node[1](x), 0, node[2]
@@ -232,11 +289,13 @@
                     b, cb, nb = x[1][:3]
                     a_up, b_up = len(x[0]) > 3, len(x[1]) > 3
                     out_hw = (b.shape[1] << b_up, b.shape[2] << b_up)
-                    x, coff, c = resize_add(a, ca, nb, out_hw, b, cb, up2=a_up, b_up2=b_up), 0, nb
+                    x, coff, c = _PendingSum(a, ca, b, cb, nb, out_hw, a_up, b_up), 0, nb
+                    if not self.fused_sums:
+                        x = x.resolve()
                 elif isinstance(ch, tuple) and ch[0] == "M":
-                    x = self._fan_out(ch[1], x, coff, c, level)
+                    x = self._fan_out(ch[1], _resolved(x), coff, c, level)
                 elif ch == "up" and i == len(items) - 1 and self.defer_up:
-                    return x, coff, c, "up2"
+                    return _resolved(x), coff, c, "up2"
                 else:
                     x, coff, c = self._run(ch, x, coff, c, level)
             return x, coff, c
@@ -253,6 +312,7 @@
             out, coff, c = self._run_fused_front(x)
         else:
             out, coff, c = self._run(self.prog, x, 0, 32)
+        out = _resolved(out)
         return out[..., coff:coff + 1].permute(0, 3, 1, 2).float()
 
     def _run_fused_front(self, x4):
```

Result: no change. 45.29 (-0.1%).
